# Tzq2doc/distributed_learning_simulator

Hardware: AMD Instinct MI355X
Metric: FL rounds/sec (FedAvg, 100 clients, ResNet-18, CIFAR-10-shaped) (higher is better)
Workload: dtype fp32; 1 GPU; fedavg_resnet18; model=ResNet18, algo=fed_avg, clients=100, local_epochs=5, global_batch=6400, per_client_batch=64, parallelism=client-dp1, backend=hip

## Files before the change

csrc/bindings.cpp:

```cpp
#include <pybind11/pybind11.h>

#include <stdexcept>
#include <string>

#include "dls.h"

namespace py = pybind11;
typedef uintptr_t ptr;

template <typename T>
static T* P(ptr p) {
  return reinterpret_cast<T*>(p);
}
static hipStream_t S(ptr s) { return reinterpret_cast<hipStream_t>(s); }

extern "C" const char* dls_src_hash();

static SgdEpi sgd_arg(const py::object& o) {
  SgdEpi e{};
  if (o.is_none()) return e;
  const py::tuple t = o.cast<py::tuple>();
  if (t.size() != 13) throw std::invalid_argument("sgd epilogue: 13 fields expected");
  e.theta = P<float>(t[0].cast<ptr>());
  e.mom = P<float>(t[1].cast<ptr>());
// ... 7 lines not shown
  e.wd = t[9].cast<float>();
  e.momentum = t[10].cast<float>();
  e.dampening = t[11].cast<float>();
  e.nesterov = t[12].cast<int>();
  return e;
}

PYBIND11_MODULE(_dls_hip, m) {
  m.doc() = "gfx950 kernels for the MI355X-native cohort FL simulator";
  m.def("src_hash", []() { return std::string(dls_src_hash()); });
  m.def("set_native_option", [](const std::string& name, int value) {
    if (!set_native_option(name.c_str(), value)) throw std::invalid_argument("unknown native option " + name);
  });

  m.def("conv_nt", [](ptr x, ptr w, ptr y, ptr bias, long x_cs, long y_cs, long w_cs, long b_cs, int B, int H, int W,
                      int C, int OH, int OW, int KH, int KW, int stride, int pad, int dil, int M, int N, int R, int rep,
                      int relu, int K, int b_kmajor, int variant, ptr acc, ptr gate, int f32, ptr s, int ldx, int ldy,
                      ptr stats, ptr stats_valid, ptr drop_seeds, float drop_p, float out_scale, ptr wsplit,
                      long ws_cs, long ws_plane, long x_lo, ptr yp, long yp_cs, long yp_lo) {
    ConvNTParams p{};
    p.yp = P<bf16_t>(yp);
    p.yp_cs = yp_cs;
    p.yp_lo = yp_lo;
    p.x_lo = x_lo;
    p.wsplit = P<const bf16_t>(wsplit);
    p.ws_cs = ws_cs;
    p.ws_plane = ws_plane;
    p.drop_seeds = P<const uint32_t>(drop_seeds);
    p.drop_p = drop_p;
    p.out_scale = out_scale;
    p.stats = P<float>(stats);
    p.stats_valid = P<const int>(stats_valid);
    p.f32 = f32;
    p.ldx = ldx;
    p.ldy = ldy;
    p.acc = P<const bf16_t>(acc);
    p.gate = P<const bf16_t>(gate);
    p.x = P<const bf16_t>(x);
    p.w = P<const bf16_t>(w);
    p.y = P<bf16_t>(y);
    p.bias = P<const bf16_t>(bias);
    p.x_cs = x_cs; p.y_cs = y_cs; p.w_cs = w_cs; p.b_cs = b_cs;
    p.B = B; p.H = H; p.W = W; p.C = C; p.OH = OH; p.OW = OW; p.KH = KH; p.KW = KW;
    p.stride = stride; p.pad = pad; p.dil = dil; p.M = M; p.N = N; p.R = R; p.rep = rep; p.relu = relu;
    p.b_kmajor = b_kmajor;
    if (stats && stats_valid && native_option(g_opt_halo_skip, "DLS_SKIP_INVALID", 1)) {
      p.skip_valid = P<const int>(stats_valid);
      p.skip_mul = OH * OW;
    }
    conv_nt(p, K, variant, S(s));
  });
  m.def("conv_dgrad", [](ptr dy, ptr w, ptr dx, ptr acc, long w_cs, int K, int rep, int B, int OH, int OW, int Co, int H,
                         int W, int Ci, int KH, int KW, int stride, int pad, int variant, int f32, ptr s, int ld_dy,
                         long dy_cs, ptr wsplit, long ws_cs, long ws_plane, long x_lo, int acc_compact, ptr bnb_part,
                         ptr bnb_x, long bnb_xld, ptr bnb_y, ptr bnb_mask, ptr bnb_mean, ptr bnb_rstd, ptr bnb_valid,
                         ptr wt_buf, ptr acc_mask, int wt_ready) {
    BNBwdPartials bnb{P<float>(bnb_part), P<const float>(bnb_x), bnb_xld, P<const float>(bnb_y),
                      P<const uint8_t>(bnb_mask), P<const float>(bnb_mean), P<const float>(bnb_rstd),
                      P<const int>(bnb_valid)};
    conv_dgrad(P<const bf16_t>(dy), P<const bf16_t>(w), P<bf16_t>(dx), P<const bf16_t>(acc), w_cs, K, rep, B, OH, OW, Co, H, W, Ci, KH, KW,
               stride, pad, variant, f32, S(s), ld_dy, dy_cs, P<const bf16_t>(wsplit), ws_cs, ws_plane, x_lo, acc_compact,
               bnb_part ? &bnb : nullptr, P<bf16_t>(wt_buf), P<const uint8_t>(acc_mask), wt_ready);
  });
  m.def("wt_planes", [](ptr wsplit, long ws_cs, long ws_plane, ptr wt, int Kw, int Co, int Ci, ptr s) {
    wt_planes(P<const bf16_t>(wsplit), ws_cs, ws_plane, P<bf16_t>(wt), Kw, Co, Ci, S(s));
  });
  m.def("conv_gl_wanted", &conv_gl_wanted);
  m.def("conv_gl_fwd", [](ptr x, ptr w, ptr y, ptr bias, long x_cs, long y_cs, long w_cs, long b_cs, int K, int rep,
                          int B, int H, int W, int C, int OH, int OW, int KH, int KW, int stride, int pad, int N,
                          int relu, ptr s) {
    conv_gl_fwd(P<const bf16_t>(x), P<const bf16_t>(w), P<bf16_t>(y), P<const bf16_t>(bias), x_cs, y_cs, w_cs, b_cs,
                K, rep, B, H, W, C, OH, OW, KH, KW, stride, pad, N, relu, S(s));
  });
  m.def("conv_weight_flip_t", [](ptr w, ptr wt, long w_cs, int Kw, int Co, int KH, int KW, int Ci, ptr s) {
    conv_weight_flip_t(P<const bf16_t>(w), P<bf16_t>(wt), w_cs, Kw, Co, KH, KW, Ci, S(s));
  });
  m.def("conv_gl_dgrad", [](ptr dy, ptr wt, ptr dx, ptr acc, int K, int rep, int B, int OH, int OW, int Co, int H, int W,
                            int Ci, int KH, int KW, int stride, int pad, ptr s) {
    conv_gl_dgrad(P<const bf16_t>(dy), P<const bf16_t>(wt), P<bf16_t>(dx), P<const bf16_t>(acc), K, rep, B, OH, OW, Co, H, W, Ci, KH, KW,
                  stride, pad, S(s));
  });
  m.def("conv_nt_num_variants", &conv_nt_num_variants);
  m.def("conv_nt_default_variant", &conv_nt_default_variant);
  m.def("conv_tn", [](ptr dy, ptr x, ptr dw, long dy_cs, long x_cs, long dw_cs, int B, int H, int W, int C, int OH,
                      int OW, int KH, int KW, int stride, int pad, int M, int Co, int R, int K, int variant, int f32,
                      ptr s, int ldy, int ldx, ptr part, long dy_lo, long x_lo, py::object sgd) {
    ConvTNParams p{};
    p.part = P<float>(part);
    p.dy_lo = dy_lo;
    p.x_lo = x_lo;
    p.f32 = f32;
    p.ldy = ldy;
    p.ldx = ldx;
    p.dy = P<const bf16_t>(dy);
    p.x = P<const bf16_t>(x);
    p.dw = P<float>(dw);
    p.dy_cs = dy_cs; p.x_cs = x_cs; p.dw_cs = dw_cs;
    p.B = B; p.H = H; p.W = W; p.C = C; p.OH = OH; p.OW = OW; p.KH = KH; p.KW = KW; p.stride = stride; p.pad = pad;
    p.M = M; p.Co = Co; p.R = R; p.splitk = 1; p.m_per_split = M;
    p.sgd = sgd_arg(sgd);
    conv_tn(p, K, variant, S(s));
  });
  m.def("conv_tn_splitk", &conv_tn_splitk, py::arg("K"), py::arg("Co"), py::arg("R"), py::arg("M"), py::arg("C"),
        py::arg("variant"), py::arg("f32"), py::arg("ldy") = 0, py::arg("ldx") = 0, py::arg("planes") = 0);
  m.def("conv_tn_pl_num_variants", &conv_tn_pl_num_variants);
  m.def("conv_tn_pl_set_variant", &conv_tn_pl_set_variant);
  m.def("conv_tn_pl_variant", &conv_tn_pl_variant);
  m.def("conv_tn_num_variants", &conv_tn_num_variants);
  m.def("conv_nt_f32_num_variants", &conv_nt_f32_num_variants);
  m.def("conv_nt_pl_num_variants", &conv_nt_pl_num_variants);
  m.def("conv_nt_pl_set_variant", &conv_nt_pl_set_variant);
  m.def("conv_halo_set_mode", &conv_halo_set_mode);
  m.def("conv_halo_set_variant", &conv_halo_set_variant);
  m.def("conv_tn_f32_num_variants", &conv_tn_f32_num_variants);

  m.def("bn_workspace_floats", &bn_workspace_floats);
  m.def("bn_fwd", [](ptr x, ptr gamma, ptr beta, ptr res, ptr y, ptr mean, ptr rstd, ptr valid, long g_cs, int K,
                     int R, int C, int relu, float eps, int rep, ptr ws, ptr mask, int f32, ptr s,
                     int ldx, ptr pre_part, int pre_nparts, ptr yp, int y_f32, ptr coef_out, int apply, ptr res_coef) {
    bn_fwd(P<const void>(x), P<const void>(gamma), P<const void>(beta), P<const void>(res), P<void>(y), P<float>(mean),
           P<float>(rstd), P<const int>(valid), g_cs, K, R, C, relu, eps, rep, P<float>(ws), P<uint8_t>(mask),
           f32, S(s), ldx, P<const float>(pre_part), pre_nparts, P<bf16_t>(yp), y_f32,
           P<float>(coef_out), apply, P<const float>(res_coef));
  });
  m.def("conv_halo_bn_supported", &conv_halo_bn_supported);
  m.def("bn_apply_only", [](ptr x, ptr coef, ptr valid, int K, int R, int C, int relu, ptr yp, ptr mask, ptr s, ptr y) {
    bn_apply_only(P<const float>(x), P<const float>(coef), P<const int>(valid), K, R, C, relu, P<bf16_t>(yp),
                  P<uint8_t>(mask), S(s), P<float>(y));
  });
  m.def("conv_halo_bn_fwd", [](ptr x, long x_cs, ptr coef, int relu, ptr valid, ptr wsplit, long ws_cs, long ws_plane,
                               int rep, ptr y, long y_cs, int K, int B, int H, int W, int C, int N, ptr stats,
                               ptr stats_valid, ptr s, ptr yp, ptr mask) {
    return conv_halo_bn_fwd(P<const float>(x), x_cs, P<const float>(coef), relu, P<const int>(valid),
                            P<const bf16_t>(wsplit), ws_cs, ws_plane, rep, P<float>(y), y_cs, K, B, H, W, C, N,
                            P<float>(stats), P<const int>(stats_valid), S(s), P<bf16_t>(yp), P<uint8_t>(mask));
  });
  m.def("bn_coef_sums", [](ptr sums, long sums_cs, int ldp, ptr gamma, ptr beta, ptr valid, long g_cs, int K, int R,
                           int C, float eps, int rep, ptr mean, ptr rstd, ptr coef, ptr s) {
    bn_coef_sums(P<const double>(sums), sums_cs, ldp, P<const float>(gamma), P<const float>(beta), P<const int>(valid),
                 g_cs, K, R, C, eps, rep, P<float>(mean), P<float>(rstd), P<float>(coef), S(s));
  });
  m.def("part_sum_f64", [](ptr part, int K, int nparts, int g, ptr out, long out_cs, int ldo, ptr s) {
    part_sum_f64(P<const float>(part), K, nparts, g, P<double>(out), out_cs, ldo, S(s));
  });
  m.def("chan_sums_f64_ws", &chan_sums_f64_ws);
  m.def("chan_sums_f64", [](ptr x, long x_cs, int ldx, int K, int R, int C, ptr valid, ptr ws, ptr out, long out_cs,
                            int ldo, ptr s) {
    chan_sums_f64(P<const float>(x), x_cs, ldx, K, R, C, P<const int>(valid), P<double>(ws), P<double>(out), out_cs, ldo,
                  S(s));
  });
  m.def("dense_wgrad_supported", &dense_wgrad_supported);
  m.def("dense_wgrad_part_floats", &dense_wgrad_part_floats);
  m.def("dense_wgrad", [](ptr dy, long dy_cs, int ldy, ptr y, long y_cs, ptr dw, long dw_cs, ptr part, int K, int B,
                          int H, int W, int C, int N, ptr s, ptr bn_sc, int ldy_x, ptr valid) {
    return dense_wgrad(P<const float>(dy), dy_cs, ldy, P<const float>(y), y_cs, P<float>(dw), dw_cs, P<float>(part), K, B,
                       H, W, C, N, S(s), P<const float>(bn_sc), ldy_x, P<const int>(valid));
  });
  m.def("dense_dgrad_supported", &dense_dgrad_supported);
  m.def("dense_dgrad_ws_floats", &dense_dgrad_ws_floats);
  m.def("dense_dgrad_bn", [](ptr dy, long dy_cs, int ldy, ptr w, long w_cs, int rep, ptr x, ptr dx, long x_cs, int ldx,
                             ptr mask, ptr y, ptr mean, ptr rstd, ptr valid, ptr gamma, long g_cs, ptr dgamma,
                             ptr dbeta, long dg_cs, ptr ws, int K, int B, int H, int W, int C, int N, ptr s,
                             ptr bn_sc) {
    DenseDgradParams p{};
    p.dy = P<const float>(dy);
    p.dy_cs = dy_cs;
    p.ldy = ldy;
    p.w = P<const float>(w);
    p.w_cs = w_cs;
    p.rep = rep;
    p.x = P<const float>(x);
    p.dx = P<float>(dx);
    p.x_cs = x_cs;
    p.ldx = ldx;
    p.mask = P<const uint8_t>(mask);
    p.y = P<const float>(y);
    p.bn_sc = P<const float>(bn_sc);
    p.mean = P<const float>(mean);
    p.rstd = P<const float>(rstd);
    p.valid_rows = P<const int>(valid);
    p.K = K;
    p.B = B;
    p.H = H;
    p.W = W;
    p.C = C;
    p.N = N;
    return dense_dgrad_bn(p, P<const float>(gamma), g_cs, P<float>(dgamma), P<float>(dbeta), dg_cs, P<float>(ws), S(s));
  });
  m.def("halo_wgrad_supported", &halo_wgrad_supported);
  m.def("halo_wgrad_part_floats", &halo_wgrad_part_floats);
  m.def("halo_wgrad", [](ptr dy, long dy_cs, long dy_lo, int ldy, ptr x, long x_cs, long x_lo, int ldx, ptr coef,
                         int relu, ptr x_valid, ptr dw, long dw_cs, ptr part, int K, int B, int H, int W, int C, int N,
                         int xm, int dm, ptr s, ptr valid_img, py::object sgd, py::object bnb) {
    HaloWgradParams p{};
    p.sgd = sgd_arg(sgd);
    if (!bnb.is_none()) {
      const py::tuple t = bnb.cast<py::tuple>();
      if (t.size() != 5) throw std::invalid_argument("halo_wgrad bnb: 5 fields expected");
      p.bb_x = P<const float>(t[0].cast<ptr>());
      p.bb_mask = P<const uint8_t>(t[1].cast<ptr>());
      p.bb_coef = P<const float>(t[2].cast<ptr>());
      p.bb_valid = P<const int>(t[3].cast<ptr>());
      p.bb_dxp = P<bf16_t>(t[4].cast<ptr>());
    }
    p.valid_img = P<const int>(valid_img);
    p.dy = P<const void>(dy);
    p.dy_cs = dy_cs;
// ... 249 lines not shown
```

csrc/conv_f32.hip:

```cpp
#include "dls.h"
#include "gemm_common.h"
#include "epilogue_f32.h"

#include <numeric>

namespace {

template <int V>
struct FV {
  float v[V];
};

template <int V>
__device__ __forceinline__ void fzero(FV<V>& f) {
#pragma unroll
  for (int i = 0; i < V; ++i) f.v[i] = 0.f;
}

template <int V>
__device__ __forceinline__ void fload(FV<V>& f, const float* p) {
  load_vec<V>(p, f.v);
}

template <int V>
// ... 253 lines not shown
        }
    }
  };

  if constexpr (NBUF == 1) {
    load();
    store(0);
    __syncthreads();
    for (int kt = 0; kt < nk; ++kt) {
      if (kt + 1 < nk) load();
      compute(0);
      if (kt + 1 < nk) {
        __syncthreads();
        store(0);
        __syncthreads();
      }
    }
  } else {
    load();
    store(0);
    __syncthreads();
    int buf = 0;
    for (int kt = 0; kt < nk; ++kt) {
      if (kt + 1 < nk) load();
      compute(buf);
      if (kt + 1 < nk) store(buf ^ 1);
      __syncthreads();
      buf ^= 1;
    }
  }

  nt_f32_epilogue<TM, TN, WM * WN, -1, false>(p, acc, smem, client, m0, n0, wm0, wn0, wid, lane);
}

template <int BM, int BN, int BK, int WM, int WN, int NBUF, int VSET, int MINW = 1>
bool launch_nt_f32_cfg(const ConvNTParams& p, int K, int va, int vb, bool bkm, hipStream_t s) {
  const int grid = K * cdiv(p.M, BM) * cdiv(p.N, BN);
  if (p.wsplit && va == 8 && vb == 8) {
    if (bkm)
      hipLaunchKernelGGL((conv_nt_f32_kernel<BM, BN, BK, WM, WN, 8, 8, true, NBUF, MINW, true>), dim3(grid),
                         dim3(WM * WN * 64), 0, s, p);
    else
      hipLaunchKernelGGL((conv_nt_f32_kernel<BM, BN, BK, WM, WN, 8, 8, false, NBUF, MINW, true>), dim3(grid),
                         dim3(WM * WN * 64), 0, s, p);
    return true;
  }
#define NTF_CASE(A, B)                                                                                       \
  if (va == A && vb == B) {                                                                                  \
    if (bkm)                                                                                                 \
      hipLaunchKernelGGL((conv_nt_f32_kernel<BM, BN, BK, WM, WN, A, B, true, NBUF, MINW>), dim3(grid),             \
                         dim3(WM * WN * 64), 0, s, p);                                                       \
    else                                                                                                     \
      hipLaunchKernelGGL((conv_nt_f32_kernel<BM, BN, BK, WM, WN, A, B, false, NBUF, MINW>), dim3(grid),            \
                         dim3(WM * WN * 64), 0, s, p);                                                       \
    return true;                                                                                             \
  }
  NTF_CASE(8, 8)
  if constexpr (VSET >= 1) { NTF_CASE(4, 4) NTF_CASE(8, 4) NTF_CASE(4, 8) }
  if constexpr (VSET >= 2) { NTF_CASE(8, 1) NTF_CASE(4, 1) NTF_CASE(1, 8) NTF_CASE(1, 4) NTF_CASE(1, 1) }
#undef NTF_CASE
  return false;
}

bool launch_nt_f32_variant(int v, const ConvNTParams& p, int K, int va, int vb, bool bkm, hipStream_t s) {
  switch (v) {
    case 0: return launch_nt_f32_cfg<128, 128, 32, 2, 2, 2, 1>(p, K, va, vb, bkm, s);
    case 1: return launch_nt_f32_cfg<128, 128, 32, 2, 2, 1, 0>(p, K, va, vb, bkm, s);
    case 2: return launch_nt_f32_cfg<256, 128, 32, 4, 2, 1, 0>(p, K, va, vb, bkm, s);
    case 3: return launch_nt_f32_cfg<64, 64, 32, 2, 2, 2, 2>(p, K, va, vb, bkm, s);
    case 4: return launch_nt_f32_cfg<128, 64, 32, 4, 1, 2, 1>(p, K, va, vb, bkm, s);
    case 5: return launch_nt_f32_cfg<128, 128, 64, 2, 2, 1, 0>(p, K, va, vb, bkm, s);
    case 6: return launch_nt_f32_cfg<256, 64, 32, 4, 1, 1, 0>(p, K, va, vb, bkm, s);
    case 7: return launch_nt_f32_cfg<64, 64, 32, 2, 2, 1, 1>(p, K, va, vb, bkm, s);
    case 8: return launch_nt_f32_cfg<128, 128, 32, 2, 2, 1, 0, 3>(p, K, va, vb, bkm, s);
    case 9: return launch_nt_f32_cfg<256, 64, 32, 4, 1, 1, 0, 3>(p, K, va, vb, bkm, s);
    case 10: return launch_nt_f32_cfg<256, 32, 32, 4, 1, 1, 1>(p, K, va, vb, bkm, s);
    default: return false;
  }
}

int vw(int c) { return (c % 8 == 0) ? 8 : (c % 4 == 0) ? 4 : 1; }


template <int BMc, int BNr, int BKT, int WM, int WN, int VA, int VB, int NBUF>
__global__ void __launch_bounds__(WM* WN * 64) conv_tn_f32_kernel(ConvTNParams p) {
  constexpr int T = WM * WN * 64;
  constexpr int TM = BMc / (WM * 32), TN = BNr / (WN * 32);
  constexpr int LDA = BMc + 32;
  constexpr int LDB = BNr + 32;
  constexpr int CCA = BMc / VA, RPA = T / CCA, PA = RPA > BKT ? 1 : BKT / RPA;
  constexpr bool A_PART = RPA > BKT;
  constexpr int CCB = BNr / VB, RPB = T / CCB, PB = BKT / RPB;
  static_assert(PA >= 1 && PB >= 1, "tile too small");
  constexpr int A_PLANE = NBUF * BKT * LDA, B_PLANE = NBUF * BKT * LDB;
  __shared__ __attribute__((aligned(16))) bf16_t smem[2 * (A_PLANE + B_PLANE)];
  bf16_t* const As = smem;
  bf16_t* const Bs = smem + 2 * A_PLANE;

  const int tid = threadIdx.x, lane = tid & 63, wid = tid >> 6;
  const int tilesM = (p.Co + BMc - 1) / BMc, tilesN = (p.R + BNr - 1) / BNr;
  const int per_client = tilesM * tilesN * p.splitk;
  const int bid = xcd_remap(blockIdx.x, gridDim.x);
  const int client = bid / per_client;
  int t = bid % per_client;
  const int split = t % p.splitk;
  t /= p.splitk;
  const int co0 = (t / tilesN) * BMc, r0 = (t % tilesN) * BNr;
  const int mbeg = split * p.m_per_split;
  const int mend = min(p.M, mbeg + p.m_per_split);

  const float* __restrict__ dy = reinterpret_cast<const float*>(p.dy) + (long)client * p.dy_cs;
  const float* __restrict__ x = reinterpret_cast<const float*>(p.x) + (long)client * p.x_cs;

  const int cb = tid % CCB;
  const int rcol = r0 + cb * VB;
  const bool rok = rcol < p.R;
  int kh = 0, kw = 0, c = 0;
  if (rok) {
    kh = rcol / (p.KW * p.C);
    const int rr = rcol - kh * p.KW * p.C;
    kw = rr / p.C;
    c = rr - kw * p.C;
  }
  const int ca = tid % CCA;
  const int cocol = co0 + ca * VA;
  const bool cok = cocol < p.Co;

  FV<VA> ra[PA];
  FV<VB> rb[PB];
  const auto dyr = make_rsrc(dy, (uint32_t)((long)p.M * p.ldy * 4));
  const auto xr = make_rsrc(x, (uint32_t)((long)p.B * p.H * p.W * p.ldx * 4));
  const bool a_live = cok && !(A_PART && tid / CCA >= BKT);
  int k_next = mbeg;
  const int q_b = BKT / (p.OH * p.OW), rem_b = BKT - q_b * p.OH * p.OW;
  const int q_oh = rem_b / p.OW, r_ow = rem_b - q_oh * p.OW;
  const int s_ldx = p.stride * p.ldx, s_row = p.stride * p.W * p.ldx, img = p.H * p.W * p.ldx;
  const int d_iw = r_ow * p.stride, d_off = r_ow * s_ldx + q_oh * s_row + q_b * img;
  const int w_wrap = p.OW * p.stride, off_c1 = s_row - p.OW * s_ldx;
  const int d_ih0 = q_oh * p.stride, d_ih1 = (q_oh + 1) * p.stride;
  const int h_wrap = p.OH * p.stride, off_c2 = img - p.OH * s_row;
  int bx_ow[PB], bx_oh[PB], bx_ih[PB], bx_iw[PB], bx_off[PB];
#pragma unroll
  for (int j = 0; j < PB; ++j) {
    const uint32_t m = mbeg + tid / CCB + j * RPB;
    const uint32_t b = fdiv(m, p.fd_ohw);
    const uint32_t rem = m - b * p.OH * p.OW;
    const uint32_t oh = fdiv(rem, p.fd_ow);
    const uint32_t ow = rem - oh * p.OW;
    bx_ow[j] = ow;
    bx_oh[j] = oh;
    bx_ih[j] = (int)oh * p.stride - p.pad + kh;
    bx_iw[j] = (int)ow * p.stride - p.pad + kw;
    bx_off[j] = (((int)b * p.H + bx_ih[j]) * p.W + bx_iw[j]) * p.ldx + c;
  }
  int a_off = (mbeg + tid / CCA) * p.ldy + cocol;
  const int a_jstep = RPA * p.ldy, a_kstep = BKT * p.ldy;
  auto load = [&]() {
    const int k0 = k_next;
    k_next += BKT;
#pragma unroll
    for (int j = 0; j < PA; ++j) {
      const int m = k0 + tid / CCA + j * RPA;
      buf_load<VA>(ra[j].v, dyr, (a_live && m < mend) ? (uint32_t)(a_off + j * a_jstep) * 4u : OOB_OFF);
    }
    a_off += a_kstep;
#pragma unroll
    for (int j = 0; j < PB; ++j) {
      const int m = k0 + tid / CCB + j * RPB;
      const bool ok = rok && m < mend && (unsigned)bx_ih[j] < (unsigned)p.H && (unsigned)bx_iw[j] < (unsigned)p.W;
      buf_load<VB>(rb[j].v, xr, ok ? (uint32_t)bx_off[j] * 4u : OOB_OFF);
      bx_ow[j] += r_ow;
      bx_iw[j] += d_iw;
      bx_off[j] += d_off;
      const bool c1 = bx_ow[j] >= p.OW;
      bx_ow[j] -= c1 ? p.OW : 0;
      bx_oh[j] += c1 ? q_oh + 1 : q_oh;
      bx_iw[j] -= c1 ? w_wrap : 0;
      bx_ih[j] += c1 ? d_ih1 : d_ih0;
      bx_off[j] += c1 ? off_c1 : 0;
      const bool c2 = bx_oh[j] >= p.OH;
      bx_oh[j] -= c2 ? p.OH : 0;
      bx_ih[j] -= c2 ? h_wrap : 0;
      bx_off[j] += c2 ? off_c2 : 0;
    }
  };
  auto store = [&](int buf) {
#pragma unroll
    for (int j = 0; j < PA; ++j) {
      if (A_PART && tid / CCA >= BKT) continue;
      const int off = (buf * BKT + tid / CCA + j * RPA) * LDA + ca * VA;
      st_split(As + off, As + A_PLANE + off, ra[j]);
    }
#pragma unroll
    for (int j = 0; j < PB; ++j) {
      const int off = (buf * BKT + tid / CCB + j * RPB) * LDB + cb * VB;
      st_split(Bs + off, Bs + B_PLANE + off, rb[j]);
    }
  };

  f32x16 acc[TM][TN];
#pragma unroll
  for (int i = 0; i < TM; ++i)
#pragma unroll
    for (int j = 0; j < TN; ++j) acc[i][j] = f32x16{};

  const int wm0 = (wid / WN) * (TM * 32), wn0 = (wid % WN) * (TN * 32);
  const int g = lane >> 4, q = (lane >> 2) & 3, pp = lane & 3, h = lane >> 5;
  auto compute = [&](int buf) {
#pragma unroll
    for (int ks = 0; ks < BKT / 16; ++ks) {
      bf16x8 ah[TM], al[TM], bh[TN], bl[TN];
      const int krow = buf * BKT + ks * 16 + 8 * h + q;
#pragma unroll
      for (int i = 0; i < TM; ++i) {
        const int o0 = krow * LDA + wm0 + i * 32 + 16 * (g & 1) + 4 * pp, o1 = o0 + 4 * LDA;
        ah[i] = tr_frag(As + o0, As + o1);
        al[i] = tr_frag(As + A_PLANE + o0, As + A_PLANE + o1);
      }
#pragma unroll
      for (int j = 0; j < TN; ++j) {
        const int o0 = krow * LDB + wn0 + j * 32 + 16 * (g & 1) + 4 * pp, o1 = o0 + 4 * LDB;
        bh[j] = tr_frag(Bs + o0, Bs + o1);
        bl[j] = tr_frag(Bs + B_PLANE + o0, Bs + B_PLANE + o1);
      }
#pragma unroll
      for (int i = 0; i < TM; ++i)
#pragma unroll
        for (int j = 0; j < TN; ++j) {
          acc[i][j] = __builtin_amdgcn_mfma_f32_32x32x16_bf16(al[i], bh[j], acc[i][j], 0, 0, 0);
          acc[i][j] = __builtin_amdgcn_mfma_f32_32x32x16_bf16(ah[i], bl[j], acc[i][j], 0, 0, 0);
          acc[i][j] = __builtin_amdgcn_mfma_f32_32x32x16_bf16(ah[i], bh[j], acc[i][j], 0, 0, 0);
        }
    }
  };

  const int nk = (mend - mbeg + BKT - 1) / BKT;
  if (nk <= 0) return;
  if constexpr (NBUF == 1) {
    load();
    store(0);
    __syncthreads();
    for (int kt = 0; kt < nk; ++kt) {
      if (kt + 1 < nk) load();
      compute(0);
      if (kt + 1 < nk) {
        __syncthreads();
        store(0);
        __syncthreads();
      }
    }
  } else {
    load();
    store(0);
    __syncthreads();
    int buf = 0;
    for (int kt = 0; kt < nk; ++kt) {
      if (kt + 1 < nk) load();
      compute(buf);
      if (kt + 1 < nk) store(buf ^ 1);
      __syncthreads();
      buf ^= 1;
    }
  }

  const bool slab = p.splitk > 1 && p.part != nullptr;
  const bool atom = p.splitk > 1 && !slab;
  float* __restrict__ dw = slab ? p.part + ((long)split * (gridDim.x / per_client) + client) * p.Co * p.R
                                : p.dw + (long)client * p.dw_cs;
#pragma unroll
  for (int j = 0; j < TN; ++j) {
    const int r = r0 + wn0 + j * 32 + (lane & 31);
#pragma unroll
    for (int i = 0; i < TM; ++i) {
#pragma unroll
      for (int e = 0; e < 16; ++e) {
        const int co = co0 + wm0 + i * 32 + (e & 3) + 8 * (e >> 2) + 4 * (lane >> 5);
        if (co < p.Co && r < p.R) {
          float* dst = dw + (long)co * p.R + r;
          if (atom)
            atomicAdd(dst, acc[i][j][e]);
          else
            *dst = acc[i][j][e];
        }
      }
    }
  }
}

template <int BMc, int BNr, int BKT, int WM, int WN, int NBUF, bool ALLV>
bool launch_tn_f32_cfg(const ConvTNParams& p, int va, int vb, int grid, hipStream_t s) {
#define TNF_CASE(A, B)                                                                                          \
  if (va == A && vb == B) {                                                                                     \
    hipLaunchKernelGGL((conv_tn_f32_kernel<BMc, BNr, BKT, WM, WN, A, B, NBUF>), dim3(grid), dim3(WM * WN * 64), \
                       0, s, p);                                                                                \
    return true;                                                                                                \
  }
  TNF_CASE(8, 8)
  if constexpr (ALLV) {
    TNF_CASE(4, 4) TNF_CASE(8, 4) TNF_CASE(4, 8) TNF_CASE(1, 1) TNF_CASE(8, 1) TNF_CASE(1, 8) TNF_CASE(4, 1)
    TNF_CASE(1, 4)
  }
#undef TNF_CASE
  return false;
}

struct TnTile {
  int bm, bn;
};
constexpr TnTile kTnF32Tiles[] = {{128, 128}, {64, 128}, {128, 128}, {256, 128}, {128, 256}, {64, 64}, {32, 128},
                                   {64, 256}};
constexpr int kTnF32Variants = sizeof(kTnF32Tiles) / sizeof(kTnF32Tiles[0]);
constexpr int TN_BKT_MAX = 32;

bool launch_tn_f32_variant(int v, const ConvTNParams& p, int va, int vb, int grid, hipStream_t s) {
  switch (v) {
    case 0: return launch_tn_f32_cfg<128, 128, 32, 2, 2, 2, true>(p, va, vb, grid, s);
    case 1: return launch_tn_f32_cfg<64, 128, 32, 2, 2, 2, true>(p, va, vb, grid, s);
    case 2: return launch_tn_f32_cfg<128, 128, 32, 2, 2, 1, false>(p, va, vb, grid, s);
    case 3: return launch_tn_f32_cfg<256, 128, 32, 4, 2, 1, false>(p, va, vb, grid, s);
    case 4: return launch_tn_f32_cfg<128, 256, 32, 2, 4, 1, false>(p, va, vb, grid, s);
    case 5: return launch_tn_f32_cfg<64, 64, 32, 2, 2, 2, true>(p, va, vb, grid, s);
    case 6: return launch_tn_f32_cfg<32, 128, 32, 1, 4, 2, true>(p, va, vb, grid, s);
    case 7: return launch_tn_f32_cfg<64, 256, 32, 2, 2, 1, false>(p, va, vb, grid, s);
    default: return false;
  }
}

int tn_f32_default_variant(int K, int Co, int R) {
  auto tiles = [&](int bm, int bn) { return (long)K * cdiv(Co, bm) * cdiv(R, bn); };
  if (Co <= 32 && R > 64) return 6;
  if (Co <= 32 || R <= 64) return 5;
  (void)tiles;
  if (R <= 256 && Co > 64) return 5;
  if (Co <= 64) return 1;
  if (Co >= 256 && R >= 2048) return 3;
  if (Co >= 1024 && R >= 512) return 3;
  return 0;
}

int resolve_tn_f32_variant(int variant, int K, int Co, int R, int va, int vb) {
  if (variant < 0 || variant >= kTnF32Variants) variant = tn_f32_default_variant(K, Co, R);
  if ((va != 8 || vb != 8) && !(variant == 0 || variant == 1 || variant == 5 || variant == 6))
    variant = Co <= 64 ? 1 : 0;
  return variant;
}

void tn_f32_split(int K, int Co, int R, int M, int variant, int& splitk, int& mps) {
  (void)K;
  const TnTile t = kTnF32Tiles[variant];
  const long tiles = (long)32 * cdiv(Co, t.bm) * cdiv(R, t.bn);
  splitk = 1;
  const int target = 1024;
  if (tiles < target) {
    splitk = (int)((target + tiles - 1) / tiles);
    splitk = min(splitk, max(1, M / (4 * TN_BKT_MAX)));
  }
  mps = cdiv(M, splitk);
  mps = ((mps + TN_BKT_MAX - 1) / TN_BKT_MAX) * TN_BKT_MAX;
  splitk = cdiv(M, mps);
}

}

int conv_nt_f32_num_variants() { return 11; }

void conv_nt_f32(const ConvNTParams& p, int K, int variant, hipStream_t s) {
  if (p.x_lo != 0) {
    if (conv_nt_pl_variant() < 0 && conv_halo(p, K, s)) return;
    if (!conv_nt_pl(p, K, conv_nt_pl_variant(), s)) {
      fprintf(stderr, "conv_nt_f32: pre-split operands in an unsupported shape (C %d, ldx %d, N %d, R %d)\n", p.C,
              p.ldx, p.N, p.R);
      abort();
    }
    return;
  }
  const bool bkm = p.b_kmajor != 0;
  const long xb = (long)p.B * p.H * p.W * p.ldx * 4;
  const long wb = (bkm ? (long)p.C * p.wKH * p.wKW * p.N : (long)p.N * p.R) * 4;
  if (p.dil != 1) {
    fprintf(stderr, "conv_nt_f32: input dilation is not supported\n");
    abort();
  }
  if (xb >= (long)OOB_OFF || wb >= (long)OOB_OFF || (p.wsplit && (p.ws_plane + wb / 4) * 2 >= (long)OOB_OFF)) {
    fprintf(stderr, "conv_nt_f32: per-client operand window over 2 GiB (x %ld B, w %ld B)\n", xb, wb);
    abort();
  }
  const int va = vw(std::gcd(p.C, p.ldx));
  int vb = bkm ? vw(p.N) : vw(p.R);
  if (variant < 0) {
    variant = p.N <= 64 ? 9 : 1;
    if (p.N <= 32) variant = 10;
    if (p.N > 64 && p.KH * p.KW == 1) variant = 8;
  }
  const bool v88 = va == 8 && vb == 8;
  const bool v84 = (va == 8 || va == 4) && (vb == 8 || vb == 4);
  if (!v88) {
    if (!v84 && variant != 3) variant = 3;
    if (v84 && !(variant == 0 || variant == 3 || variant == 4 || variant == 7 || variant == 10))
      variant = p.N <= 64 ? 4 : 0;
  }
  if (!launch_nt_f32_variant(variant, p, K, va, vb, bkm, s)) fprintf(stderr, "conv_nt_f32: bad variant %d\n", variant);
  if (p.yp) {
    if (p.yp_cs != 2 * p.y_cs || p.yp_lo != p.y_cs || p.ldy != p.N || p.out_s != 1) {
      fprintf(stderr, "conv_nt_f32: output planes need contiguous per-client rows\n");
      abort();
    }
    split_rows(reinterpret_cast<const float*>(p.y), p.yp, K, (long)p.M * p.N, p.y_cs, s);
  }
}

int conv_tn_f32_num_variants() { return kTnF32Variants; }

void conv_tn_f32(ConvTNParams p, int K, int variant, hipStream_t s) {
  if (p.sgd.theta && p.dy_lo == 0) {
    fprintf(stderr, "conv_tn_f32: the SGD epilogue needs pre-split operands\n");
    abort();
  }
  if (p.dy_lo != 0) {
    if (!conv_tn_pl(p, K, variant, s)) {
      fprintf(stderr, "conv_tn_f32: pre-split operands in an unsupported shape (C %d, Co %d)\n", p.C, p.Co);
      abort();
    }
    return;
  }
  const long dyb = (long)p.M * (p.ldy ? p.ldy : p.Co) * 4, xb = (long)p.B * p.H * p.W * (p.ldx ? p.ldx : p.C) * 4;
  if (dyb >= (long)OOB_OFF || xb >= (long)OOB_OFF) {
    fprintf(stderr, "conv_tn_f32: per-client operand window over 2 GiB (dy %ld B, x %ld B)\n", dyb, xb);
    abort();
  }
  const int va = vw(std::gcd(p.Co, p.ldy));
  const int vb = vw(std::gcd(p.C, p.ldx));
  variant = resolve_tn_f32_variant(variant, K, p.Co, p.R, va, vb);
  tn_f32_split(K, p.Co, p.R, p.M, variant, p.splitk, p.m_per_split);
  const TnTile t = kTnF32Tiles[variant];
  const long tiles = (long)K * cdiv(p.Co, t.bm) * cdiv(p.R, t.bn);
  const int grid = (int)(tiles * p.splitk);
  if (!launch_tn_f32_variant(variant, p, va, vb, grid, s)) fprintf(stderr, "conv_tn_f32: bad variant %d\n", variant);
  if (p.splitk > 1 && p.part != nullptr) tn_fold(p.part, p.dw, p.dw_cs, K, p.splitk, (long)p.Co * p.R, s);
}

int conv_tn_f32_splitk(int K, int Co, int R, int M, int gco, int gc, int variant) {
  int splitk, mps;
  variant = resolve_tn_f32_variant(variant, K, Co, R, vw(gco), vw(gc));
  tn_f32_split(K, Co, R, M, variant, splitk, mps);
  return splitk;
}
```

csrc/dls.h:

```cpp
#pragma once
#include <hip/hip_runtime.h>
#include <stdint.h>

typedef uint16_t bf16_t;

constexpr int kOptUnset = -1000000;
extern int g_opt_attn_mfma, g_opt_conv_gl, g_opt_pl_min_wg;
extern int g_opt_halo_wgrad_unroll;
extern int g_opt_halo_skip;
extern int g_opt_conv_pix;
int native_option(int& slot, const char* env, int dflt);
bool set_native_option(const char* name, int value);

struct FastDiv {
  uint32_t d, mul, shift;
};

static inline FastDiv make_fastdiv(uint32_t d) {
  FastDiv f;
  f.d = d;
  uint32_t s = 0;
  while ((1u << s) < d) ++s;
  f.shift = s;
  f.mul = (uint32_t)((((uint64_t)1 << 32) * (((uint64_t)1 << s) - d)) / d + 1);
// ... 84 lines not shown
  float* part;
  int K, B, H, W, C, N, nchunks, G;
  const float* bn_sc;
  int ldy_x;
  const int* valid_rows;
};

struct DenseDgradParams {
  const float* dy;
  long dy_cs;
  int ldy;
  const float* w;
  long w_cs;
  int rep;
  const float* x;
  float* dx;
  long x_cs;
  int ldx;
  const uint8_t* mask;
  const float* y;
  const float* bn_sc;
  const float* mean;
  const float* rstd;
  const int* valid_rows;
  const float* coef;
  float* part;
  int K, B, H, W, C, N, G, nchunks;
};

struct SgdEpi {
  float* theta;
  float* mom;
  bf16_t* split;
  long th_cs, sp_cs, sp_lo;
  const float* lr;
  const uint8_t* active;
  const uint8_t* first;
  float wd, momentum, dampening;
  int nesterov;
};

struct HaloWgradParams {
  const void* dy;
  long dy_cs, dy_lo;
  int ldy;
  const void* x;
  long x_cs, x_lo;
  int ldx;
  const float* coef;
  int relu;
  const int* x_valid;
  const int* valid_img;
  const float* bb_x;
  const uint8_t* bb_mask;
  const float* bb_coef;
  const int* bb_valid;
  bf16_t* bb_dxp;
  float* dw;
  long dw_cs;
  float* part;
  int K, B, H, W, C, N;
  int nblk, cblk, G;
  SgdEpi sgd;
};
bool halo_wgrad_supported(int B, int H, int W, int C, int N);
long halo_wgrad_part_floats(int K, int B, int H, int W, int C, int N);
bool halo_wgrad(HaloWgradParams p, int xm, int dm, hipStream_t s);

struct ConvTNParams {
  const bf16_t* dy;
  const bf16_t* x;
  float* dw;
  long dy_cs, x_cs, dw_cs;
  int B, H, W, C, OH, OW, KH, KW, stride, pad;
  int M, Co, R;
  int splitk, m_per_split;
  FastDiv fd_ohw, fd_ow;
  int f32;
  int ldy, ldx;
  float* part;
  long dy_lo, x_lo;
  SgdEpi sgd;
  int pix;
};

struct ConvGLParams {
  const bf16_t* x;
  const bf16_t* w;
  bf16_t* y;
  const bf16_t* bias;
  const bf16_t* acc;
  const bf16_t* zero;
  long x_cs, y_cs, w_cs, b_cs;
  int B, H, W, C;
  int OH, OW;
  int stride, pad_h, pad_w;
  int M, N, ldb, ntaps, cchunks;
  int tap_dh[9], tap_dw[9], tap_boff[9];
  int rep, relu;
  int out_s, out_ph, out_pw, out_H, out_W;
  FastDiv fd_ohw, fd_ow;
};
bool conv_gl_supported(int C, int N, int ntaps);
bool conv_gl_wanted(int K, int M, int N, int C, int ntaps, int mode);
void conv_gl_fwd(const bf16_t* x, const bf16_t* w, bf16_t* y, const bf16_t* bias, long x_cs, long y_cs, long w_cs,
                 long b_cs, int K, int rep, int B, int H, int W, int C, int OH, int OW, int KH, int KW, int stride,
                 int pad, int N, int relu, hipStream_t s);
void conv_weight_flip_t(const bf16_t* w, bf16_t* wt, long w_cs, int Kw, int Co, int KH, int KW, int Ci,
                        hipStream_t s);
void conv_gl_dgrad(const bf16_t* dy, const bf16_t* wt, bf16_t* dx, const bf16_t* acc, int K, int rep, int B, int OH, int OW, int Co,
                   int H, int W, int Ci, int KH, int KW, int stride, int pad, hipStream_t s);

void conv_nt(ConvNTParams p, int K, int variant, hipStream_t s);
int conv_nt_num_variants();
int conv_nt_default_variant(int M, int N, int R, int b_kmajor);
void conv_dgrad(const bf16_t* dy, const bf16_t* w, bf16_t* dx, const bf16_t* acc, long w_cs, int K, int rep, int B, int OH, int OW,
                int Co, int H, int W, int Ci, int KH, int KW, int stride, int pad, int variant, int f32, hipStream_t s,
                int ld_dy = 0, long dy_cs = 0, const bf16_t* wsplit = nullptr, long ws_cs = 0, long ws_plane = 0,
                long x_lo = 0, int acc_compact = 0,
                const BNBwdPartials* bnb = nullptr,
                bf16_t* wt_buf = nullptr,
                const uint8_t* acc_mask = nullptr,
                int wt_ready = 0);
void wt_planes(const bf16_t* wsplit, long ws_cs, long ws_plane, bf16_t* wt, int Kw, int Co, int Ci, hipStream_t s);
void conv_tn(ConvTNParams p, int K, int variant, hipStream_t s);
int conv_tn_num_variants();
int conv_tn_splitk(int K, int Co, int R, int M, int C, int variant, int f32, int ldy = 0, int ldx = 0,
                   int planes = 0);
void conv_nt_f32(const ConvNTParams& p, int K, int variant, hipStream_t s);
int conv_nt_f32_num_variants();
void conv_tn_f32(ConvTNParams p, int K, int variant, hipStream_t s);
bool conv_nt_pl_supported(const ConvNTParams& p);
bool conv_nt_pl(const ConvNTParams& p, int K, int variant, hipStream_t s);
int conv_nt_pl_num_variants();
int conv_nt_pl_variant();
void conv_nt_pl_set_variant(int v);
bool conv_halo(const ConvNTParams& p, int K, hipStream_t s);
bool conv_halo_bn_supported(int B, int H, int W, int C, int N);
void bn_coef_sums(const double* sums, long sums_cs, int ldp, const float* gamma, const float* beta,
                  const int* valid_rows, long g_cs, int K, int R, int C, float eps, int rep, float* mean, float* rstd,
                  float* coef, hipStream_t s);
void part_sum_f64(const float* part, int K, int nparts, int g, double* out, long out_cs, int ldo, hipStream_t s);
long chan_sums_f64_ws(int R, int C);
void chan_sums_f64(const float* x, long x_cs, int ldx, int K, int R, int C, const int* valid, double* ws, double* out,
                   long out_cs, int ldo, hipStream_t s);
void bn_apply_only(const float* x, const float* coef, const int* valid_rows, int K, int R, int C, int relu,
                   bf16_t* yp, uint8_t* rmask, hipStream_t s, float* y = nullptr);
bool conv_halo_bn_fwd(const float* x, long x_cs, const float* coef, int relu, const int* valid_rows,
                      const bf16_t* wsplit, long ws_cs, long ws_plane, int rep, float* y, long y_cs, int K, int B,
                      int H, int W, int C, int N, float* stats, const int* stats_valid, hipStream_t s,
                      bf16_t* yp = nullptr, uint8_t* mask = nullptr);
bool conv_halo_bn_dense_supported(int B, int H, int W, int C, int N);
bool conv_halo_bn_dense_fwd(const float* x, long x_cs, int ldx, int creal, const float* coef, int relu,
                            const int* valid_rows, const bf16_t* wsplit, long ws_cs, long ws_plane, int rep, float* y,
                            long y_cs, int ldy, int K, int B, int H, int W, int C, int N, float* stats,
                            const int* stats_valid, float* ny, long ny_cs, int ldny, uint8_t* mask, hipStream_t s);
bool dense_dgrad_supported(int B, int H, int W, int C, int N);
long dense_dgrad_ws_floats(int K, int B, int H, int C);
bool dense_dgrad_bn(DenseDgradParams p, const float* gamma, long g_cs, float* dgamma, float* dbeta, long dg_cs,
                    float* ws, hipStream_t s);
void bn_bwd_coef_parts(const float* part, int nparts, const float* gamma, long g_cs, const int* valid_rows,
                       const float* mean, const float* rstd, int K, int R, int C, float* coef, float* dgamma,
                       float* dbeta, long dg_cs, hipStream_t s);
bool dense_wgrad_supported(int B, int H, int W, int C, int N);
long dense_wgrad_part_floats(int K, int B, int H, int W, int C);
bool dense_wgrad(const float* dy, long dy_cs, int ldy, const float* y, long y_cs, float* dw, long dw_cs, float* part,
                 int K, int B, int H, int W, int C, int N, hipStream_t s, const float* bn_sc = nullptr,
                 int ldy_x = 0, const int* valid_rows = nullptr);
void conv_halo_set_mode(int m);
void conv_halo_set_variant(int v);
bool conv_tn_pl_supported(const ConvTNParams& p);
bool conv_tn_pl(ConvTNParams p, int K, int variant, hipStream_t s);
int conv_tn_pl_num_variants();
int conv_tn_pl_variant();
void conv_tn_pl_set_variant(int v);
int conv_tn_pl_splitk(int K, int Co, int R, int M, int variant);
void tn_fold(const float* part, float* dw, long dw_cs, int K, int splitk, long CoR, hipStream_t s,
             const SgdEpi* sgd = nullptr);
int conv_tn_f32_num_variants();
int conv_tn_f32_splitk(int K, int Co, int R, int M, int gco, int gc, int variant);

long bn_workspace_floats(int K, long R, int C);
void bn_fwd(const void* x, const void* gamma, const void* beta, const void* res, void* y, float* mean, float* rstd,
            const int* valid_rows, long g_cs, int K, int R, int C, int relu, float eps, int rep, float* ws,
            uint8_t* relu_mask, int f32, hipStream_t s,
            int ldx = 0, const float* pre_part = nullptr,
            int pre_nparts = 0, bf16_t* yp = nullptr,
            int y_f32 = 1, float* coef_out = nullptr, int apply = 1,
            const float* res_coef = nullptr);
void bn_bwd(const void* dy, const void* x, const void* y, const float* mean, const float* rstd, const void* gamma,
            const int* valid_rows, long g_cs, int K, int R, int C, int relu, void* dx, void* dpre, float* dgamma,
            float* dbeta, long dg_cs, float* ws, const uint8_t* relu_mask, int f32,
            hipStream_t s, int ldx = 0,
            int acc_dx = 0, bf16_t* dxp = nullptr,
            int dx_f32 = 1,
            const float* pre_part = nullptr,
            int pre_nparts = 0,
            float* coef_ext = nullptr,
            int stage = 0);
void ln_fwd(const void* x, const void* gamma, const void* beta, void* y, float* mean, float* rstd, long g_cs, int K,
            long rows_per_client, int C, float eps, int rep, int f32, hipStream_t s,
            bf16_t* yp = nullptr);
void ln_bwd(const void* dy, const void* x, const float* mean, const float* rstd, const void* gamma, long g_cs, int K,
            long rows_per_client, int C, void* dx, float* dgamma, float* dbeta, long dg_cs, float* ws, int f32,
            hipStream_t s);
long col_sum_workspace_floats(int K, long rows, int C);
long ln_workspace_floats(int K, long rows_per_client, int C);
void col_sum(const void* x, float* out, long out_cs, int K, long rows, int C, int f32, hipStream_t s,
             float* ws = nullptr);

void pool_fwd(const void* x, void* y, int* idx, int K, int B, int H, int W, int C, int OH, int OW, int k, int stride,
              int pad, int mode, int f32, hipStream_t s);
void pool_bwd(const void* dy, const int* idx, void* dx, int K, int B, int H, int W, int C, int OH, int OW, int k,
              int stride, int pad, int mode, int f32, hipStream_t s);
void gap_fwd(const void* x, void* y, int KB, int HW, int C, int f32, hipStream_t s);
void gap_bwd(const void* dy, void* dx, int KB, int HW, int C, int f32, hipStream_t s);
void ce_fwd_bwd(const void* logits, const int* labels, const int* valid, float* loss, float* correct, void* dlogits,
                int K, int B, int NC, int f32, hipStream_t s, float* rowbuf = nullptr);
void relu_bwd(const void* dy, const void* y, void* dx, long n, int f32, hipStream_t s);

void quant_pack(const float* x, long ld, const int* seg, const int64_t* seg_off, const int64_t* seg_numel,
                const uint8_t* bits, const float* lo, const float* scale, const int64_t* seg_byte_off,
                const int64_t* row_off, int K, int nseg, long P, int stochastic, const uint32_t* seeds, uint8_t* out,
                hipStream_t s);
void quant_unpack(const uint8_t* codes, const int* seg, const int64_t* seg_off, const int64_t* seg_numel,
                  const uint8_t* bits, const float* lo, const float* scale, const int64_t* seg_byte_off,
                  const int64_t* row_off, int K, int nseg, long P, float* out, long ld, hipStream_t s);
void quant_unpack_acc(const uint8_t* codes, const int* seg, const int64_t* seg_off, const int64_t* seg_numel,
                      const uint8_t* bits, const float* lo, const float* scale, const int64_t* seg_byte_off,
                      const int64_t* row_off, int K, int nseg, long P, const double* w, double* acc, hipStream_t s);

#define TOPK_CHUNK 4096
void topk_pack(const float* delta, long ld_d, float* u, long ld_u, int ef, const uint32_t* vbits, uint32_t* hist,
               uint32_t* state, uint32_t* cnt, uint32_t* excl, int* idx, float* val, int K, long P, int k,
               hipStream_t s);
void topk_decode(const int* idx, const float* val, float* out, long ld, int K, long P, int k, hipStream_t s);
void topk_accumulate(const int* idx, const float* val, const double* w, double* acc, int K, long P, int k,
                     hipStream_t s);

#define TRIM_MAX_ROWS 512
void trimmed_sum(const float* x, long ld, int n, int b, long P, double* out, hipStream_t s);

#define PAIR_SPAN 4096
#define PAIR_GROUP 8
int pairwise_spans_per_wg(int n, long P);
long pairwise_ws_doubles(int n, long P, int spw);
void pairwise_sq_dists(const float* x, long ld, int n, long P, double* ws, int spw, double* out, hipStream_t s);

void dropout_apply(const void* x, void* out, int K, long rows, int N, long ld, const uint32_t* seeds, float p,
                   float scale, int f32, hipStream_t s);
long dropout_planes_ws_floats(int K, long rows, int N);
void dropout_planes(const float* x, float* out, bf16_t* yp, int K, long rows, int N, const uint32_t* seeds, float p,
                    float scale, hipStream_t s, float* colsum = nullptr, long colsum_cs = 0, float* ws = nullptr);
void fold_col_partials(const float* part, int nparts, int C, float* out, long out_cs, int K, hipStream_t s);

void synth_images(const int64_t* idx, long n, long npix, int C, int Cout, const int* source, const float* proto,
                  unsigned long long salt, float sqrt6, float noise, float* out, hipStream_t s);

void neighbor_sample(const int* rowptr, const int* col, const int* owner, const uint8_t* is_val, const int64_t* nodes,
                     const int64_t* clients, int n, int fanout, unsigned long long seed_h, int* out_nbr, int* out_cnt,
                     hipStream_t s);

void sgd_step(float* theta, const float* grad, float* mom, bf16_t* shadow, bf16_t* split, const float* lr,
              const uint8_t* active,
              const uint8_t* first, int K, long P, long ld, float wd, float momentum, float dampening, int nesterov,
              hipStream_t s);
void sgd_step_seg(float* theta, const float* grad, float* mom, bf16_t* split, const float* lr, const uint8_t* active,
                  const uint8_t* first, int K, long ld, float wd, float momentum, float dampening, int nesterov,
                  const long2* seg, int nblocks, hipStream_t s);
void adam_step(float* theta, const float* grad, float* m, float* v, bf16_t* shadow, const float* lr,
               const uint8_t* active, const float* step, int K, long P, long ld, float b1, float b2, float eps,
               float wd, hipStream_t s);
// ... 50 lines not shown
```

csrc/norm.hip:

```cpp
#include "common.h"
#include <algorithm>
#include <numeric>

#include "dls.h"

namespace {

constexpr int ROWS_PER_BLOCK = 512;

static int rows_per_block(long R, int K) {
  const long want = std::min<long>(64, (2048 + K - 1) / K);
  const long bpc = std::max(1L, std::min(want, std::max(1L, R / 64)));
  return (int)std::min<long>(ROWS_PER_BLOCK, (R + bpc - 1) / bpc);
}

struct BNCoefArgs {
  const void* gamma;
  const void* beta;
  const float* mean_in;
  const float* rstd_in;
  float* mean_out;
  float* rstd_out;
  float* coef;
  float* dgamma;
// ... 244 lines not shown
  if (c < C) {
    const int lp = ldp ? ldp : C;
    const PT* part = ws + (long)k * (pcs ? pcs : (long)nparts * 2 * lp);
    for (int b = grp; b < nparts; b += G) {
      d0 += part[(long)b * 2 * lp + c];
      d1 += part[(long)b * 2 * lp + lp + c];
    }
  }
  red[0][grp][cl] = d0;
  red[1][grp][cl] = d1;
  __syncthreads();
  if (grp != 0 || c >= C) return;
#pragma unroll
  for (int g2 = 1; g2 < G; ++g2) {
    d0 += red[0][g2][cl];
    d1 += red[1][g2][cl];
  }
  const float s0 = (float)d0, s1 = (float)d1;
  const long i = (long)k * C + c;
  const int nvalid = valid_rows ? min(valid_rows[k], R) : R;
  const float n = (float)max(nvalid, 1);
  const float g = ldf(gamma + (long)(k / rep) * g_cs + c);
  if (!bwd) {
    const double mud = d0 / n;
    const float mu = (float)mud;
    const float var = (float)fmax(d1 / n - mud * mud, 0.0);
    const float rs = rsqrtf(var + eps);
    const float sc = g * rs;
    mean_out[i] = mu;
    rstd_out[i] = rs;
    coef[2 * i] = sc;
    coef[2 * i + 1] = ldf(beta + (long)(k / rep) * g_cs + c) - mu * sc;
  } else {
    const float mu = mean_in[i], rs = rstd_in[i];
    const float a = g * rs;
    const float e = -a * rs * s1 / n;
    const float d = -a * s0 / n - e * mu;
    coef[3 * i] = a;
    coef[3 * i + 1] = d;
    coef[3 * i + 2] = e;
    if (dgamma) {
      dbeta[(long)k * dg_cs + c] = s0;
      dgamma[(long)k * dg_cs + c] = s1;
    }
  }
}

template <typename TT, typename PT, typename... A>
void launch_coef(dim3 grid, hipStream_t s, A... args) {
  hipLaunchKernelGGL((bn_coef_kernel<TT, PT, 8>), grid, dim3(32 * 8), 0, s, args...);
}

template <int V>
__device__ __forceinline__ void store_planes(bf16_t* hi, bf16_t* lo, const float* f) {
  if constexpr (V % 2 == 0) {
    uint32_t h[V / 2], l[V / 2];
#pragma unroll
    for (int i = 0; i < V / 2; ++i) split_pair(f[2 * i], f[2 * i + 1], h[i], l[i]);
    if constexpr (V == 8) {
      *reinterpret_cast<uint4*>(hi) = make_uint4(h[0], h[1], h[2], h[3]);
      *reinterpret_cast<uint4*>(lo) = make_uint4(l[0], l[1], l[2], l[3]);
    } else if constexpr (V == 4) {
      *reinterpret_cast<uint2*>(hi) = make_uint2(h[0], h[1]);
      *reinterpret_cast<uint2*>(lo) = make_uint2(l[0], l[1]);
    } else {
#pragma unroll
      for (int i = 0; i < V / 2; ++i) {
        reinterpret_cast<uint32_t*>(hi)[i] = h[i];
        reinterpret_cast<uint32_t*>(lo)[i] = l[i];
      }
    }
  } else {
#pragma unroll
    for (int i = 0; i < V; ++i) split2(f[i], hi[i], lo[i]);
  }
}

template <typename T, int V>
__global__ void __launch_bounds__(256) bn_apply_kernel(const T* __restrict__ x, const T* __restrict__ res,
                                                       T* __restrict__ y, const int* __restrict__ valid_rows,
                                                       const float* __restrict__ coef, int R, int C, int relu,
                                                       int rpb, uint8_t* __restrict__ rmask, int ldx,
                                                       bf16_t* __restrict__ yp, int y_f32,
                                                       const float* __restrict__ res_coef) {
  const int k = blockIdx.y;
  const int CT = C / V;
  const int nvalid = valid_rows ? min(valid_rows[k], R) : R;
  const int r0 = blockIdx.x * rpb, r1 = min(R, r0 + rpb);
  const long base = (long)k * R * C, base_x = (long)k * R * ldx;
  for (int cg = 0; cg < CT; cg += 256) {
    const int ctn = min(256, CT - cg);
    const int RT = 256 / ctn;
    const int cc = threadIdx.x % ctn, rl = threadIdx.x / ctn;
    if (rl >= RT) continue;
    const int c0 = (cg + cc) * V;
    float sc[V], sh[V], rsc[V], rsh[V];
#pragma unroll
    for (int j = 0; j < V; ++j) {
      sc[j] = coef[2 * ((long)k * C + c0 + j)];
      sh[j] = coef[2 * ((long)k * C + c0 + j) + 1];
      rsc[j] = res_coef ? res_coef[2 * ((long)k * C + c0 + j)] : 0.f;
      rsh[j] = res_coef ? res_coef[2 * ((long)k * C + c0 + j) + 1] : 0.f;
    }
    for (int r = r0 + rl; r < r1; r += RT) {
      const long off = base + (long)r * C + c0;
      float out[V];
      if (r < nvalid) {
        float v[V];
        const long offx = base_x + (long)r * ldx + c0;
        load_vec<V>(x + offx, v);
#pragma unroll
        for (int j = 0; j < V; ++j) out[j] = fmaf(v[j], sc[j], sh[j]);
        if (res) {
          float rv[V];
          load_vec<V>(res + offx, rv);
          if (res_coef) {
#pragma unroll
            for (int j = 0; j < V; ++j) out[j] += fmaf(rv[j], rsc[j], rsh[j]);
          } else {
#pragma unroll
            for (int j = 0; j < V; ++j) out[j] += rv[j];
          }
        }
        if (relu) {
#pragma unroll
          for (int j = 0; j < V; ++j) out[j] = fmaxf(out[j], 0.f);
        }
      } else {
#pragma unroll
        for (int j = 0; j < V; ++j) out[j] = 0.f;
      }
      if (rmask) {
        uint32_t m = 0;
#pragma unroll
        for (int j = 0; j < V; ++j) m |= (rt<T>(out[j]) > 0.f ? 1u : 0u) << j;
        rmask[((long)k * R + r) * (C / 8) + c0 / 8] = (uint8_t)m;
      }
      if (y_f32) store_vec<V>(y + off, out);
      if (yp) {
        bf16_t* hp = yp + (long)k * R * C + off;
        store_planes<V>(hp, hp + (long)R * C, out);
      }
    }
  }
}

template <typename T, int V>
__global__ void __launch_bounds__(256) bn_bwd_apply_kernel(const T* __restrict__ dy, const T* __restrict__ x,
                                                           const T* __restrict__ y,
                                                           const int* __restrict__ valid_rows,
                                                           const float* __restrict__ coef, int R, int C, int relu,
                                                           T* __restrict__ dx, T* __restrict__ dpre,
                                                           int rpb, const uint8_t* __restrict__ rmask, int ldx,
                                                           int acc_dx, bf16_t* __restrict__ dxp, int dx_f32) {
  const int k = blockIdx.y;
  const int CT = C / V;
  const int nvalid = valid_rows ? min(valid_rows[k], R) : R;
  const int r0 = blockIdx.x * rpb, r1 = min(R, r0 + rpb);
  const long base = (long)k * R * C, base_x = (long)k * R * ldx;
  for (int cg = 0; cg < CT; cg += 256) {
    const int ctn = min(256, CT - cg);
    const int RT = 256 / ctn;
    const int cc = threadIdx.x % ctn, rl = threadIdx.x / ctn;
    if (rl >= RT) continue;
    const int c0 = (cg + cc) * V;
    float ca[V], cd[V], ce[V];
#pragma unroll
    for (int j = 0; j < V; ++j) {
      const long q = 3 * ((long)k * C + c0 + j);
      ca[j] = coef[q];
      cd[j] = coef[q + 1];
      ce[j] = coef[q + 2];
    }
    for (int r = r0 + rl; r < r1; r += RT) {
      const long off = base + (long)r * C + c0;
      const long offx = base_x + (long)r * ldx + c0;
      float o[V], gp[V];
      if (r < nvalid) {
        float vdy[V], vx[V];
        load_vec<V>(dy + off, vdy);
        load_vec<V>(x + offx, vx);
        if (rmask) {
          const uint32_t mbits = rmask[((long)k * R + r) * (C / 8) + c0 / 8];
#pragma unroll
          for (int j = 0; j < V; ++j) vdy[j] = ((mbits >> j) & 1u) ? vdy[j] : 0.f;
        } else if (relu) {
          float vy[V];
          load_vec<V>(y + off, vy);
#pragma unroll
          for (int j = 0; j < V; ++j) vdy[j] = vy[j] > 0.f ? vdy[j] : 0.f;
        }
#pragma unroll
        for (int j = 0; j < V; ++j) {
          gp[j] = vdy[j];
          o[j] = fmaf(ca[j], vdy[j], fmaf(ce[j], vx[j], cd[j]));
        }
      } else {
#pragma unroll
        for (int j = 0; j < V; ++j) o[j] = gp[j] = 0.f;
// ... 157 lines not shown
    b = wave_sum(b) / C;
#pragma unroll
    for (int i = 0; i < NC; ++i) {
      const int c = lane + 64 * i;
      if (c < C) stf(dx + row * C + c, crs * (cy[i] * gv[i] - a - xh[i] * b));
    }
#pragma unroll
    for (int i = 0; i < NC; ++i) {
      cy[i] = ny[i];
      cx[i] = nx[i];
    }
    cmu = nmu;
    crs = nrs;
  }
  if (rend > rbeg || part) {
#pragma unroll
    for (int i = 0; i < NC; ++i) {
      const int c = lane + 64 * i;
      if (c < C) {
        if (part) {
          float* pw = part + ((long)k * gridDim.x * 4 + wave) * 2 * C;
          pw[c] = dg[i];
          pw[C + c] = db[i];
        } else {
          atomicAdd(&dgamma[(long)k * dg_cs + c], dg[i]);
          atomicAdd(&dbeta[(long)k * dg_cs + c], db[i]);
        }
      }
    }
  }
}

__global__ void __launch_bounds__(256) part_sum_kernel(const float* __restrict__ part, int nparts, int W, int C,
                                                       float* __restrict__ out0, float* __restrict__ out1, long out_cs) {
  const int k = blockIdx.y, c = blockIdx.x * 256 + threadIdx.x;
  if (c >= C) return;
  const float* p = part + (long)k * nparts * W;
  float a = 0.f, b = 0.f;
  for (int i = 0; i < nparts; ++i) {
    a += p[(long)i * W + c];
    if (out1) b += p[(long)i * W + C + c];
  }
  out0[(long)k * out_cs + c] = a;
  if (out1) out1[(long)k * out_cs + c] = b;
}

}

#define DISPATCH_V(V, ...)          \
  if (V == 8) {                     \
    constexpr int VV = 8;           \
    __VA_ARGS__;                    \
  } else if (V == 4) {              \
    constexpr int VV = 4;           \
    __VA_ARGS__;                    \
  } else {                          \
    constexpr int VV = 1;           \
    __VA_ARGS__;                    \
  }
#define DISPATCH_T(F32, ...)        \
  if (F32) {                        \
    typedef float TT;               \
    __VA_ARGS__;                    \
  } else {                          \
    typedef bf16_t TT;              \
    __VA_ARGS__;                    \
  }
#define CP(p) static_cast<const TT*>(p)
#define MP(p) static_cast<TT*>(p)

static long bn_fold_offset(int K, long R, int C) {
  const long parts = (R + rows_per_block(R, K) - 1) / rows_per_block(R, K);
  return ((long)K * 3 * C + (long)K * parts * 2 * C + 1) & ~1L;
}

long bn_workspace_floats(int K, long R, int C) {
  const long nfold = cdiv((int)cdiv((int)R, 32), FOLD);
  return bn_fold_offset(K, R, C) + (long)K * nfold * 2 * C * 2;
}

void bn_fwd(const void* x, const void* gamma, const void* beta, const void* res, void* y, float* mean, float* rstd,
            const int* valid_rows, long g_cs, int K, int R, int C, int relu, float eps, int rep, float* ws,
            uint8_t* rmask, int f32, hipStream_t s, int ldx, const float* pre_part,
            int pre_nparts, bf16_t* yp, int y_f32, float* coef_out, int apply, const float* res_coef) {
  if (ldx == 0) ldx = C;
  float* coef = coef_out ? coef_out : ws;
  const float* part = pre_part ? pre_part : ws + (long)3 * C * K;
  const int rpb = rows_per_block(R, K);
  dim3 grid(cdiv(R, rpb), K);
  const int nparts = pre_part ? pre_nparts : (int)grid.x;
  const int V = vw(std::gcd(C, ldx));
  BNCoefArgs ca{gamma, beta, nullptr, nullptr, mean, rstd, coef, nullptr, nullptr, 0L, g_cs, eps, rep, 0};
  if (V != 8) rmask = nullptr;
  DISPATCH_T(f32, {
    if (!pre_part) {
      DISPATCH_V(V, hipLaunchKernelGGL((chan_reduce_kernel<TT, VV, 0>), grid, dim3(256), 0, s, CP(x), nullptr, nullptr,
                                       nullptr, nullptr, valid_rows, R, C, 0, ws + (long)3 * C * K, (long)2 * C, rpb,
                                       nullptr, ca, ldx, ldx));
    }
    if (pre_part && nparts > FOLD && nparts <= cdiv(R, 32)) {
      const int nfold = cdiv(nparts, FOLD);
      double* folds = reinterpret_cast<double*>(ws + bn_fold_offset(K, R, C));
      hipLaunchKernelGGL(part_fold_kernel, dim3(nfold, K), dim3(256), 0, s, pre_part, nparts, 2 * C, folds, nfold);
      launch_coef<TT, double>(dim3(cdiv(C, 32), K), s, (const double*)folds, nfold, CP(gamma), CP(beta), valid_rows,
                              (const float*)nullptr, (const float*)nullptr, mean, rstd, coef, (float*)nullptr,
                              (float*)nullptr, 0L, g_cs, K, R, C, eps, rep, 0, 0, 0L);
    } else {
      launch_coef<TT, float>(dim3(cdiv(C, 32), K), s, part, nparts, CP(gamma), CP(beta), valid_rows,
                             (const float*)nullptr, (const float*)nullptr, mean, rstd, coef, (float*)nullptr,
                             (float*)nullptr, 0L, g_cs, K, R, C, eps, rep, 0, 0, 0L);
    }
    if (apply) {
      DISPATCH_V(V, hipLaunchKernelGGL((bn_apply_kernel<TT, VV>), grid, dim3(256), 0, s, CP(x), CP(res), MP(y),
                                       valid_rows, coef, R, C, relu, rpb, rmask, ldx, f32 ? yp : nullptr,
                                       f32 ? y_f32 : 1, res_coef));
    }
  });
}

void bn_apply_only(const float* x, const float* coef, const int* valid_rows, int K, int R, int C, int relu,
                   bf16_t* yp, uint8_t* rmask, hipStream_t s, float* y) {
  const int rpb = rows_per_block(R, K);
  dim3 grid(cdiv(R, rpb), K);
  if (C % 8 == 0) {
    hipLaunchKernelGGL((bn_apply_kernel<float, 8>), grid, dim3(256), 0, s, x, (const float*)nullptr, y,
                       valid_rows, coef, R, C, relu, rpb, rmask, C, yp, y ? 1 : 0, (const float*)nullptr);
  } else {
    hipLaunchKernelGGL((bn_apply_kernel<float, 1>), grid, dim3(256), 0, s, x, (const float*)nullptr, y,
                       valid_rows, coef, R, C, relu, rpb, (uint8_t*)nullptr, C, yp, y ? 1 : 0, (const float*)nullptr);
  }
}

void bn_bwd(const void* dy, const void* x, const void* y, const float* mean, const float* rstd, const void* gamma,
            const int* valid_rows, long g_cs, int K, int R, int C, int relu, void* dx, void* dpre, float* dgamma,
            float* dbeta, long dg_cs, float* ws, const uint8_t* rmask, int f32, hipStream_t s,
            int ldx, int acc_dx, bf16_t* dxp, int dx_f32, const float* pre_part, int pre_nparts, float* coef_ext,
            int stage) {
  if (!f32 || acc_dx || (ldx != 0 && ldx != C)) {
    dxp = nullptr;
    dx_f32 = 1;
  }
  if (ldx == 0) ldx = C;
  float* coef = coef_ext ? coef_ext : ws;
  float* part = ws + (long)3 * C * K;
  const int rpb = rows_per_block(R, K);
  dim3 grid(cdiv(R, rpb), K);
  const int V = vw(std::gcd(C, ldx));
  if (V != 8) rmask = nullptr;
  BNCoefArgs ca{gamma, nullptr, mean, rstd, nullptr, nullptr, coef, dgamma, dbeta, dg_cs, g_cs, 0.f, 1, 1};
  DISPATCH_T(f32, {
    if (stage == 2) {
    } else if (pre_part) {
      if (pre_nparts > FOLD && pre_nparts <= cdiv(R, 32)) {
        const int nfold = cdiv(pre_nparts, FOLD);
        double* folds = reinterpret_cast<double*>(ws + bn_fold_offset(K, R, C));
        hipLaunchKernelGGL(part_fold_kernel, dim3(nfold, K), dim3(256), 0, s, pre_part, pre_nparts, 2 * C, folds,
                           nfold);
        launch_coef<TT, double>(dim3(cdiv(C, 32), K), s, (const double*)folds, nfold, CP(gamma), (const TT*)nullptr,
                                valid_rows, mean, rstd, (float*)nullptr, (float*)nullptr, coef, dgamma, dbeta, dg_cs,
                                g_cs, K, R, C, 0.f, 1, 1, 0, 0L);
      } else {
        launch_coef<TT, float>(dim3(cdiv(C, 32), K), s, pre_part, pre_nparts, CP(gamma), (const TT*)nullptr,
                               valid_rows, mean, rstd, (float*)nullptr, (float*)nullptr, coef, dgamma, dbeta, dg_cs,
                               g_cs, K, R, C, 0.f, 1, 1, 0, 0L);
      }
    } else {
      DISPATCH_V(V, hipLaunchKernelGGL((chan_reduce_kernel<TT, VV, 1>), grid, dim3(256), 0, s, CP(dy), CP(x), CP(y),
                                       mean, rstd, valid_rows, R, C, relu, part, (long)2 * C, rpb, rmask, ca, C, ldx));
    }
    if (!pre_part && stage != 2)
      launch_coef<TT, float>(dim3(cdiv(C, 32), K), s, (const float*)part, (int)grid.x, CP(gamma), (const TT*)nullptr,
                             valid_rows, mean, rstd, (float*)nullptr, (float*)nullptr, coef, dgamma, dbeta, dg_cs, g_cs, K,
                             R, C, 0.f, 1, 1, 0, 0L);
    if (stage != 1)
      DISPATCH_V(V, hipLaunchKernelGGL((bn_bwd_apply_kernel<TT, VV>), grid, dim3(256), 0, s, CP(dy), CP(x), CP(y),
                                       valid_rows, coef, R, C, relu, MP(dx), MP(dpre), rpb, rmask, ldx, acc_dx, dxp,
                                       dx_f32));
  });
}

void fold_col_partials(const float* part, int nparts, int C, float* out, long out_cs, int K, hipStream_t s) {
  hipLaunchKernelGGL(part_sum_kernel, dim3(cdiv(C, 256), K), dim3(256), 0, s, part, nparts, C, C, out, (float*)nullptr,
                     out_cs);
}

void bn_bwd_coef_parts(const float* part, int nparts, const float* gamma, long g_cs, const int* valid_rows,
                       const float* mean, const float* rstd, int K, int R, int C, float* coef, float* dgamma,
                       float* dbeta, long dg_cs, hipStream_t s) {
  launch_coef<float, float>(dim3(cdiv(C, 32), K), s, part, nparts, gamma, (const float*)nullptr, valid_rows, mean, rstd,
                            (float*)nullptr, (float*)nullptr, coef, dgamma, dbeta, dg_cs, g_cs, K, R, C, 0.f, 1, 1, 0,
                            0L);
}

void part_sum_f64(const float* part, int K, int nparts, int g, double* out, long out_cs, int ldo, hipStream_t s) {
  if (K == 0) return;
  hipLaunchKernelGGL(part_sum_f64_kernel<float>, dim3(K), dim3(1024), 0, s, part, nparts, g, out, out_cs, ldo);
}

long chan_sums_f64_ws(int R, int C) { return (long)cdiv(R, 256) * 2 * C; }

void chan_sums_f64(const float* x, long x_cs, int ldx, int K, int R, int C, const int* valid, double* ws, double* out,
                   long out_cs, int ldo, hipStream_t s) {
  if (K == 0 || R == 0) return;
  const int rb = 256, nch = cdiv(R, rb);
  hipLaunchKernelGGL(chan_sums_f64_kernel, dim3(nch, K), dim3(256), 0, s, x, x_cs, ldx, R, C, valid, rb, ws, nch);
  hipLaunchKernelGGL(part_sum_f64_kernel<double>, dim3(K), dim3(1024), 0, s, (const double*)ws, nch, C, out, out_cs,
                     ldo);
}

void bn_coef_sums(const double* sums, long sums_cs, int ldp, const float* gamma, const float* beta,
                  const int* valid_rows, long g_cs, int K, int R, int C, float eps, int rep, float* mean, float* rstd,
                  float* coef, hipStream_t s) {
// ... 74 lines not shown
```

distributed_learning_simulator_amd/models/zoo.py:

```python

from __future__ import annotations

import math

import torch

from ..engine.params import ParamLayout
from ..ops import functional as Fn
from .layers import (AvgPool, BatchNorm, Conv2d, Embedding, conv_bn, Flatten, LayerNorm, Linear,
                     MaxPool, Module, ReLU, RunCtx, Seq)


class CohortModel:

    def __init__(self, root: Module, name: str, input_kind: str, num_classes: int):
        self.root = root
        self.name = name
        self.input_kind = input_kind
        self.num_classes = num_classes
        root.assign_names("")
        self.layout = ParamLayout()
        root.register(self.layout)

    def forward(self, x, ctx: RunCtx):
# ... 55 lines not shown
        return Fn.ResidualLink()
    return None


def _down(seq: Seq, x, ctx, donor=None):
    conv, bn = seq.children
    return conv_bn(conv, bn, x, ctx, conv_donor=donor, planes=4)


class BasicBlock(Module):
    kind = "BasicBlock"
    expansion = 1

    def __init__(self, cin, cout, stride):
        super().__init__()
        self.child("conv1", Conv2d(cin, cout, 3, stride, 1))
        self.child("bn1", BatchNorm(cout, relu=True))
        self.child("conv2", Conv2d(cout, cout, 3, 1, 1))
        self.child("bn2", BatchNorm(cout))
        self.down = None
        if stride != 1 or cin != cout:
            self.down = self.child("downsample", Seq(Conv2d(cin, cout, 1, stride, 0), BatchNorm(cout)))

    def forward(self, x, ctx, out_planes: int = 1):
        link = _residual_link(self, x, ctx)
        out = conv_bn(self.conv1, self.bn1, x, ctx, conv_link=link, planes=3)
        sc = x if self.down is None else _down(self.down, x, ctx, donor=link)
        return conv_bn(self.conv2, self.bn2, out, ctx, residual=sc, relu=True,
                       link=link if self.down is None else None, planes=out_planes)


class Bottleneck(Module):
    kind = "Bottleneck"
    expansion = 4

    def __init__(self, cin, width, stride):
        super().__init__()
        cout = width * 4
        self.child("conv1", Conv2d(cin, width, 1, 1, 0))
        self.child("bn1", BatchNorm(width, relu=True))
        self.child("conv2", Conv2d(width, width, 3, stride, 1))
        self.child("bn2", BatchNorm(width, relu=True))
        self.child("conv3", Conv2d(width, cout, 1, 1, 0))
        self.child("bn3", BatchNorm(cout))
        self.down = None
        if stride != 1 or cin != cout:
            self.down = self.child("downsample", Seq(Conv2d(cin, cout, 1, stride, 0), BatchNorm(cout)))

    def forward(self, x, ctx, out_planes: int = 1):
        link = _residual_link(self, x, ctx)
        out = conv_bn(self.conv1, self.bn1, x, ctx, conv_link=link, planes=2)
        out = conv_bn(self.conv2, self.bn2, out, ctx, planes=2)
        sc = x if self.down is None else _down(self.down, x, ctx, donor=link)
        return conv_bn(self.conv3, self.bn3, out, ctx, residual=sc, relu=True,
                       link=link if self.down is None else None, planes=out_planes)


class ResNetNet(Module):
    kind = "ResNet"

    def __init__(self, block, layers, classes=10, cin=3, cifar_stem=True):
        super().__init__()
        self.cifar_stem = cifar_stem
        if cifar_stem:
            self.child("conv1", Conv2d(cin, 64, 3, 1, 1))
        else:
            self.child("conv1", Conv2d(cin, 64, 7, 2, 3))
        self.child("bn1", BatchNorm(64, relu=True))
        if not cifar_stem:
            self.child("maxpool", MaxPool(3, 2, 1))
        c = 64
        self.stages = []
        for i, (n, w) in enumerate(zip(layers, (64, 128, 256, 512))):
            blocks = []
            for j in range(n):
                stride = 2 if (j == 0 and i > 0) else 1
                b = block(c, w, stride)
                blocks.append(b)
                c = w * block.expansion
            self.stages.append(self.child(f"layer{i + 1}", Seq(*blocks)))
        self.child("fc", Linear(c, classes))

    def forward(self, x, ctx):
        x = conv_bn(self.conv1, self.bn1, x, ctx, planes=0 if not self.cifar_stem else 1)
        if not self.cifar_stem:
            x = self.maxpool.forward(x, ctx)
        blocks = [b for s in self.stages for b in s.children]
        for i, b in enumerate(blocks):
            nxt = blocks[i + 1] if i + 1 < len(blocks) else None
            op = 0 if nxt is None else 2 if nxt.down is not None else 1
            x = b.forward(x, ctx, out_planes=op)
        x = Fn.global_avg_pool(x)
        return self.fc.forward(x, ctx)


class DenseLayer(Module):

    kind = "DenseLayer"

    def __init__(self, cin, growth):
        super().__init__()
        self.child("norm", BatchNorm(cin, relu=True))
        self.child("relu", ReLU())
        self.child("conv", Conv2d(cin, growth, 3, 1, 1))

    def forward(self, x, ctx):
        y = self.conv.forward(self.norm.forward(x, ctx), ctx)
        return torch.cat([x, y], dim=-1)


class Transition(Module):
    kind = "Transition"

    def __init__(self, cin, cout):
        super().__init__()
        self.child("norm", BatchNorm(cin, relu=True))
        self.child("relu", ReLU())
        self.child("conv", Conv2d(cin, cout, 1, 1, 0))
        self.child("pool", AvgPool(2))

    def forward(self, x, ctx):
        return self.pool.forward(self.conv.forward(self.norm.forward(x, ctx), ctx), ctx)


class DenseBlock(Seq):

    kind = "Sequential"

    def __init__(self, layers, growth):
        super().__init__(*layers)
        self.growth = growth

    def forward(self, x, ctx):
        P = ctx.P
        lps = [Fn.DenseLayerParams(P.w(l.norm.gamma), P.w(l.norm.beta), P.g(l.norm.gamma), P.g(l.norm.beta),
                                   P.w(l.conv.w), P.g(l.conv.w)) for l in self.children]
        rps = x.shape[2] * x.shape[3]
        return Fn.dense_block(x, ctx.token, lps, self.growth, ctx.valid_rows(rps), training=ctx.training)


class DenseNetNet(Module):
    kind = "DenseNet"

    def __init__(self, depth=40, growth=12, classes=10, cin=3):
        super().__init__()
        n = (depth - 4) // 3
        c = 2 * growth
        self.child("conv1", Conv2d(cin, c, 3, 1, 1))
        self.blocks = []
        for b in range(3):
            layers = []
            for _ in range(n):
                layers.append(DenseLayer(c, growth))
                c += growth
            self.blocks.append(self.child(f"dense{b + 1}", DenseBlock(layers, growth)))
            if b < 2:
                self.blocks.append(self.child(f"trans{b + 1}", Transition(c, c)))
        self.child("norm", BatchNorm(c, relu=True))
        self.child("relu", ReLU())
        self.child("fc", Linear(c, classes))

    def forward(self, x, ctx):
        x = self.conv1.forward(x, ctx)
        for b in self.blocks:
            x = b.forward(x, ctx)
        x = self.norm.forward(x, ctx)
        x = Fn.global_avg_pool(x)
        return self.fc.forward(x, ctx)


# ... 220 lines not shown
```

distributed_learning_simulator_amd/ops/functional.py:

```python

from __future__ import annotations

import collections

import torch

from ..options import OPTIONS
from . import backend, ref


def _be(t):
    return backend.get(t)


class ResidualLink:

    __slots__ = ("grad", "receiver_done", "compact", "receiver_stride")

    def __init__(self):
        self.grad = None
        self.receiver_done = False
        self.compact = 0
        self.receiver_stride = 1


class MaskedGrad:

    __slots__ = ("dy", "mask")

    def __init__(self, dy, mask):
        self.dy, self.mask = dy, mask

    def dense(self):
        K, C = self.dy.shape[0], self.dy.shape[-1]
        bits = torch.arange(8, device=self.mask.device, dtype=torch.uint8)
        keep = ((self.mask.view(K, -1, C // 8, 1) >> bits) & 1).reshape(K, -1, C).bool()
        return torch.where(keep, self.dy.reshape(K, -1, C), torch.zeros((), dtype=self.dy.dtype,
                                                                          device=self.dy.device)).view(self.dy.shape)




class BNStats:

    __slots__ = ("valid", "part", "dy_planes_ok")

    def __init__(self, valid=None):
        self.valid = valid
        self.part = None
        self.dy_planes_ok = False


bn_bwd_parts_count = {"used": 0, "none": 0, "fallback": 0}


class BNBwdLink:

    __slots__ = ("x", "mask", "mean", "rstd", "valid", "part", "key")

    def __init__(self, x, mask, mean, rstd, valid):
        self.x, self.mask, self.mean, self.rstd, self.valid = x, mask, mean, rstd, valid
        self.part = None
        self.key = None

    def args(self, part):
        return (part, self.x, self.mask, self.mean, self.rstd, self.valid, None)




def _planes_of(t):
    return getattr(t, "_dls_planes", None)


def _tag_planes(t, planes, only: bool):
    t._dls_planes = planes
    t._dls_planes_only = only
    return t


def _require_fp32(t, who: str):
    if getattr(t, "_dls_planes_only", False):
        raise RuntimeError(f"{who}: a planes-only activation reached an op that reads fp32 values")


class DeferredBN:

    __slots__ = ("x", "coef", "relu", "valid_rows", "yp", "mask", "write_out", "pending")

    def __init__(self, x, coef, relu, valid_rows, yp, mask, write_out):
        self.x, self.coef, self.relu, self.valid_rows = x, coef, relu, valid_rows
        self.yp, self.mask, self.write_out = yp, mask, write_out
        self.pending = True

    def materialize(self):
        if self.pending:
            from . import hip

            hip.bn_apply_only(self.x, self.coef, self.valid_rows, self.relu, self.yp, self.mask)
            self.pending = False


res_fold_count = {"folded": 0, "materialized": 0}


class DeferredRes:

    __slots__ = ("x", "coef", "valid_rows", "y", "pending")

    def __init__(self, x, coef, valid_rows, y):
        self.x, self.coef, self.valid_rows, self.y = x, coef, valid_rows, y
        self.pending = True

    def materialize(self):
        if self.pending:
            from . import hip

            hip.bn_apply_only(self.x, self.coef, self.valid_rows, False, None, y=self.y)
            self.pending = False
            res_fold_count["materialized"] += 1


bn_bwd_defer_count = {"wgrad": 0, "materialized": 0}


class DeferredBNBwd:

    __slots__ = ("dy", "x", "mask", "coef", "valid_rows", "dxp", "pending")

    def __init__(self, dy, x, mask, coef, valid_rows, dxp):
        self.dy, self.x, self.mask, self.coef, self.valid_rows, self.dxp = dy, x, mask, coef, valid_rows, dxp
        self.pending = True

    def materialize(self):
        if self.pending:
            from . import hip

            hip.bn_bwd_apply_planes(self.dy, self.x, self.mask, self.coef, self.valid_rows, self.dxp)
            self.pending = False
            bn_bwd_defer_count["materialized"] += 1

    def wgrad_args(self):
        return (self.dy, self.x, self.mask, self.coef, self.valid_rows, self.dxp)


class _Conv(torch.autograd.Function):

    @staticmethod
    def forward(ctx, x, token, w, gw, stride, pad, b, gb, link=None, stats=None, w_split=None, donor=None,
                sgd=None):
        be = _be(x)
        ci = w.shape[-1]
        ctx.sgd = sgd if (sgd is not None and be is not ref and x.dtype == torch.float32 and gw is not None
                          and b is None and x.shape[-1] == ci and w_split is not None) else None
        if x.shape[-1] > ci:
            w = torch.nn.functional.pad(w, (0, x.shape[-1] - ci))
            w_split = None
        if be is ref or x.dtype != torch.float32:
            w_split = None
        xp = _planes_of(x)
        use_pl = (xp is not None and w_split is not None and x.is_contiguous()
                  and be.conv_planes_ok(x.shape[-1], w.shape[1]) and be.planes_fit(x[0].numel()))
        if getattr(x, "_dls_planes_only", False) and not use_pl:
            raise RuntimeError("conv2d: planes-only input but the split-plane GEMM cannot run here")
        pl = {"x_planes": xp} if use_pl else {}
        ctx.xp = xp if use_pl else None
        if stats is not None:
            stats.dy_planes_ok = use_pl and b is None
        K, B, H, W = x.shape[:4]
        KH = w.shape[2]
        OH, OW = (H + 2 * pad - KH) // stride + 1, (W + 2 * pad - w.shape[3]) // stride + 1
        y_numel = B * OH * OW * w.shape[1]
        big = be is not ref and max(x[0].numel(), y_numel) * x.element_size() >= (1 << 31)
        if stats is not None:
            stats.dy_planes_ok = stats.dy_planes_ok and be.planes_fit(y_numel)
        want_stats = stats is not None and be is not ref and x.dtype == torch.float32 and not big
        y = None
        ctx.bn_src = None
        defer = getattr(x, "_dls_bn_defer", None)
        if defer is not None and defer.pending:
            if (use_pl and stride == 1 and pad == 1 and KH == 3 and w.shape[3] == 3 and b is None
                    and be.halo_bn_ok(x.shape, w)):
                part = (torch.empty((K, be.conv_stats_parts(B * OH * OW), 2, w.shape[1]), dtype=torch.float32,
                                    device=x.device) if want_stats else None)
                bn_wgrad = (defer.write_out and gw is not None and OPTIONS.halo_wgrad
                            and x.shape[-1] == ci and be.halo_wgrad_ok(x.shape, w.shape[1]))
                y = be.conv_halo_bn_fwd(defer.x.view(x.shape), defer.coef, defer.relu, defer.valid_rows, w, w_split,
                                        stats=part, stats_valid=stats.valid if want_stats else None,
                                        yp=defer.yp if defer.write_out and not bn_wgrad else None,
                                        mask=defer.mask if defer.write_out else None)
                if y is not None:
                    defer.pending = False
                    if want_stats:
                        stats.part = part
                    if bn_wgrad:
                        ctx.bn_src = (defer.x.view(x.shape), defer.coef, defer.relu, defer.valid_rows)
            defer.materialize()
        if y is not None:
            pass
        elif want_stats:
            stats.part = torch.empty((K, be.conv_stats_parts(B * OH * OW), 2, w.shape[1]), dtype=torch.float32,
                                     device=x.device)
            y = be.conv_fwd(x, w, stride, pad, bias=b, stats=stats.part, stats_valid=stats.valid,
                            **({"w_split": w_split} if w_split is not None else {}), **pl)
        elif w_split is not None:
            y = be.conv_fwd(x, w, stride, pad, bias=b, w_split=w_split, **pl)
        else:
            y = be.conv_fwd(x, w, stride, pad, bias=b)
        ctx.w_split = w_split
        ctx.expect_dy_planes = stats is not None and stats.dy_planes_ok
        ctx.x_planes_only = bool(getattr(x, "_dls_planes_only", False))
        bnb = getattr(x, "_dls_bnb", None) if OPTIONS.bn_bwd_parts else None
        if bnb is not None and not (be is not ref and donor is None and x.shape[-1] == ci and not big
                                    and be.bn_bwd_parts_ok(x.shape, stride, x.dtype)):
            bnb = None
        ctx.bnb = bnb
        ctx.halo_wgrad = OPTIONS.halo_wgrad
        ctx.valid = stats.valid if (stats is not None and OPTIONS.skip_invalid) else None
        ctx.dgrad_wt = be is not ref
        ctx.save_for_backward(x, w)
        ctx.gw, ctx.gb, ctx.stride, ctx.pad, ctx.ci = gw, gb, stride, pad, ci
        ctx.link = link
        ctx.donor = donor
        if link is not None:
            link.receiver_stride = stride
        return y

    @staticmethod
    def _wgrad(ctx, dy, x, w, dyp, be, bbd=None, sgd_ok=True) -> bool:
        if bbd is not None:
            if not (ctx.stride == 1 and ctx.pad == 1 and w.shape[2] == 3 and w.shape[3] == 3):
                return False
            sgd = ctx.sgd if sgd_ok else None
            if ctx.bn_src is not None:
                xr, coef, relu, vrows = ctx.bn_src
                ok = be.halo_wgrad(dy, xr, ctx.gw, bn=(coef, relu, vrows), valid=ctx.valid, sgd=sgd,
                                   bn_bwd=bbd.wgrad_args())
            else:
                ok = be.halo_wgrad(dy, x, ctx.gw, x_planes=ctx.xp, valid=ctx.valid, sgd=sgd, bn_bwd=bbd.wgrad_args())
            if ok and sgd is not None:
                sgd[0].done.add(sgd[1])
            return bool(ok)
        padded = w.shape[-1] > ctx.ci
        K = x.shape[0]
        sgd = ctx.sgd if not padded else None
        stepped = False
        gw = torch.empty((K,) + tuple(w.shape[1:]), dtype=torch.float32, device=dy.device) if padded else ctx.gw
        if be is ref:
            gw.copy_(ref.conv_wgrad(dy.float(), x.float(), (K,) + tuple(w.shape[1:]), ctx.stride, ctx.pad))
            if ctx.gb is not None:
                ctx.gb.copy_(dy.float().sum(dim=(1, 2, 3)))
        elif ctx.bn_src is not None:
            xr, coef, relu, vrows = ctx.bn_src
            if not be.halo_wgrad(dy, xr, gw, dy_planes=dyp, bn=(coef, relu, vrows), valid=ctx.valid,
                                 sgd=sgd):
                raise RuntimeError("conv2d backward: the halo wgrad refused a shape its forward accepted")
            stepped = sgd is not None
        elif (ctx.halo_wgrad and ctx.stride == 1 and ctx.pad == 1 and w.shape[2] == 3 and w.shape[3] == 3
              and not padded and be.halo_wgrad(dy, x, gw, dy_planes=dyp, x_planes=ctx.xp, valid=ctx.valid,
                                               sgd=sgd)):
            stepped = sgd is not None
        elif dyp is not None:
            stepped = be.conv_wgrad(dy, x, gw, ctx.stride, ctx.pad, dy_planes=dyp, x_planes=ctx.xp, sgd=sgd)
        else:
            if ctx.x_planes_only:
                raise RuntimeError("conv2d backward: fp32 dY with a planes-only input")
            be.conv_wgrad(dy, x, gw, ctx.stride, ctx.pad)
            if ctx.gb is not None:
                be.bias_grad(dy, ctx.gb)
        if padded:
            ctx.gw.copy_(gw[..., : ctx.ci])
        if stepped:
            sgd[0].done.add(sgd[1])
        return True

    @staticmethod
    def backward(ctx, dy):
        x, w = ctx.saved_tensors
        be = _be(dy)
        dy = dy.contiguous()
        dx = None
        link = ctx.link
        acc = link.grad if link is not None else None
        acc_mask = None
        if isinstance(acc, MaskedGrad):
            if be is not ref and dy.dtype == torch.float32 and ctx.needs_input_grad[0] and not link.compact:
                acc, acc_mask = acc.dy.contiguous(), acc.mask
            else:
                acc = acc.dense()
        acc_compact = False
        if link is not None:
            if acc is not None and link.compact:
                if link.compact == ctx.stride and ctx.stride > 1 and be is not ref and ctx.needs_input_grad[0]:
                    acc_compact = True
                else:
                    full = torch.zeros(x.shape, dtype=acc.dtype, device=acc.device)
                    full[:, :, :: link.compact, :: link.compact] = acc
                    acc = full
            link.grad = None
            link.compact = 0
            if acc is None:
                link.receiver_done = True
        dyp = _planes_of(dy)
        wgrad_done = False
        wt_pre = None
        bbd = getattr(dy, "_dls_bnbwd", None)
        if bbd is not None and bbd.pending:
            if ctx.gw is not None and be is not ref and ctx.halo_wgrad and w.shape[-1] == ctx.ci:
                sgd_ok = True
                if ctx.sgd is not None and ctx.needs_input_grad[0]:
                    wt_pre = (be.dgrad_wt_prebuild(dy.shape, w, ctx.w_split, x.shape[2:4], ctx.stride, ctx.pad)
                              if ctx.dgrad_wt and ctx.w_split is not None and not acc_compact and ctx.donor is None
                              else None)
                    sgd_ok = wt_pre is not None
                wgrad_done = _Conv._wgrad(ctx, dy, x, w, dyp, be, bbd, sgd_ok=sgd_ok)
            if wgrad_done:
                bbd.pending = False
                bn_bwd_defer_count["wgrad"] += 1
            else:
                bbd.materialize()
        if dyp is not None and ctx.xp is None:
            raise RuntimeError("conv2d backward: dY planes without the input's planes")
        if dyp is None:
            if ctx.expect_dy_planes:
                raise RuntimeError("conv2d backward: the BN wrote dY as planes only, but they did not arrive")
            _require_fp32(dy, "conv2d backward")
        donor = ctx.donor
        compact = (donor is not None and not donor.receiver_done and be is not ref and dy.dtype == torch.float32
                   and ctx.stride > 1 and ctx.pad == 0 and w.shape[2] == 1 and w.shape[3] == 1 and acc is None
                   and w.shape[-1] == ctx.ci and donor.receiver_stride == ctx.stride)
        if ctx.needs_input_grad[0] and compact:
            dx = be.conv_dgrad(dy, w, dy.shape[2:4], 1, 0, w_split=ctx.w_split,
                               **({"dy_planes": dyp} if dyp is not None else {}))
        elif ctx.needs_input_grad[0]:
            if acc_compact:
                dx = be.conv_dgrad(dy, w, x.shape[2:4], ctx.stride, ctx.pad, acc=acc, w_split=ctx.w_split,
                                   acc_compact=True, **({"dy_planes": dyp} if dyp is not None else {}))
            else:
                kw = {}
                bnb = ctx.bnb
                if bnb is not None:
                    K, B, H, W, Ci = x.shape
                    part = torch.empty((K, be.conv_stats_parts(B * H * W), 2, Ci), dtype=torch.float32,
                                       device=dy.device)
                    kw["bnb"] = bnb.args(part)
                if dyp is not None:
                    kw["dy_planes"] = dyp
                if ctx.w_split is not None:
                    kw["w_split"] = ctx.w_split
                if acc_mask is not None:
                    kw["acc_mask"] = acc_mask
                if ctx.dgrad_wt:
                    kw["wt"] = True
                if wt_pre is not None:
                    kw["wt_buf"] = wt_pre
                dx = be.conv_dgrad(dy, w, x.shape[2:4], ctx.stride, ctx.pad, acc=acc, **kw)
                if bnb is not None:
                    bnb.part, bnb.key = part, (dx.data_ptr(), dx._version)
            if dx.shape[-1] > ctx.ci:
                dx = dx[..., : ctx.ci]
        elif acc is not None:
            dx = acc if acc_mask is None else MaskedGrad(acc, acc_mask).dense()
        if ctx.gw is not None and not wgrad_done:
            _Conv._wgrad(ctx, dy, x, w, dyp, be)
        if donor is not None and dx is not None and not donor.receiver_done:
            donor.grad = dx
            donor.compact = ctx.stride if compact else 0
            dx = None
        return dx, None, None, None, None, None, None, None, None, None, None, None, None


def conv2d(x, token, w, gw, stride=1, pad=0, b=None, gb=None, link: ResidualLink | None = None,
           stats: BNStats | None = None, w_split: torch.Tensor | None = None, donor: ResidualLink | None = None,
           sgd=None):
    if link is not None:
        assert w.shape[-1] == x.shape[-1], "a residual link needs an unpadded conv"
    return _Conv.apply(x, token, w, gw, stride, pad, b, gb, link, stats, w_split, donor, sgd)


class _Linear(torch.autograd.Function):

    @staticmethod
    def forward(ctx, x, token, w, b, gw, gb, residual=None, relu=False, premasked=False, gate_input=False,
                drop_p=0.0, drop_seeds=None, gate_scale=1.0, w_split=None, x_planes=None, out_planes=False,
                dx_planes=False, res_link=None, acc_link=None, sgd=None):
        be = _be(x)
        ctx.res_link, ctx.acc_link = res_link, acc_link
        shp = x.shape
        x = x.reshape(shp[0], -1, shp[-1])
        ctx.res_shape = residual.shape if residual is not None else None
        if residual is not None:
            residual = residual.reshape(shp[0], x.shape[1], -1).contiguous()
        native = be is not ref and x.dtype == torch.float32 and w_split is not None and OPTIONS.planes
        if not native:
            w_split = x_planes = None
            out_planes = dx_planes = False
        if not OPTIONS.tfm_planes:
            out_planes = dx_planes = False
        ws = {"w_split": w_split} if w_split is not None else {}
        xp = {"x_planes": x_planes} if x_planes is not None else {}
        y = be.linear_fwd(x, w, b, relu=relu, acc=residual, drop_p=drop_p, drop_seeds=drop_seeds, **ws, **xp,
                          **({"out_planes": True} if out_planes else {}))
        yp = None
        if out_planes:
            y, yp = y
        ctx.ws = ws
        mask_dy = relu and not premasked
        ctx.save_for_backward(x, w, y if mask_dy else None, drop_seeds if drop_p else None)
        ctx.x_planes = x_planes
# ... 54 lines not shown
            if dyp is not None:
                kw["dy_planes"] = dyp
            if ctx.dx_planes:
                kw["out_planes"] = True
            if acc is not None and be is not ref:
                kw["acc"] = acc.reshape(K, N, Fi)
            dx = be.linear_dgrad(dy, w, gate=gate, gate_scale=ctx.gate_scale, **kw)
            dxp = None
            if ctx.dx_planes:
                dx, dxp = dx
            if acc is not None and be is ref:
                dx = dx + acc.reshape(dx.shape)
            dx = dx.view(ctx.shape)
            if dxp is not None:
                _tag_planes(dx, dxp.view((K, 2) + tuple(ctx.shape[1:])), False)
        if ctx.gw is not None:
            if be is ref:
                dw, db = ref.linear_wgrad(dy.float(), x.float(), ctx.gb is not None)
                ctx.gw.copy_(dw)
                if ctx.gb is not None:
                    ctx.gb.copy_(db)
            else:
                pl = {"dy_planes": dyp, "x_planes": ctx.x_planes} if (dyp is not None and ctx.x_planes is not None) else {}
                if pl and ctx.sgd is not None:
                    pl["sgd"] = ctx.sgd
                if be.linear_wgrad(dy, x, ctx.gw, None if bias_done else ctx.gb, **pl):
                    ctx.sgd[0].done.add(ctx.sgd[1])
        if dx is None and acc is not None:
            dx = acc.reshape(ctx.shape)
        return (dx, None, None, None, None, None, dres, None, None, None, None, None, None, None, None, None, None, None,
                None, None)


def linear(x, token, w, b, gw, gb, residual=None, relu=False, premasked=False, gate_input=False,
           drop_p: float = 0.0, drop_seeds=None, gate_scale: float = 1.0, w_split=None, out_planes: bool = False,
           dx_planes: bool = False, res_link: ResidualLink | None = None, acc_link: ResidualLink | None = None,
           sgd=None):
    assert not (relu and residual is not None), "ReLU and residual epilogues are not combined"
    return _Linear.apply(x, token, w, b, gw, gb, residual, relu, premasked, gate_input, drop_p, drop_seeds,
                         gate_scale, w_split, _planes_of(x), out_planes, dx_planes, res_link, acc_link, sgd)


class _LinearSharedInput(torch.autograd.Function):

    @staticmethod
    def forward(ctx, x, token, w, gw):
        be = _be(x)
        K, Fo, Fi = w.shape
        wcat = w.reshape(1, K * Fo, Fi).contiguous()
        y = be.linear_fwd(x.unsqueeze(0).contiguous(), wcat, None)
        ctx.save_for_backward(x)
        ctx.gw, ctx.K, ctx.Fo = gw, K, Fo
        return y[0].view(-1, K, Fo).permute(1, 0, 2).contiguous()

    @staticmethod
    def backward(ctx, dy):
        (x,) = ctx.saved_tensors
        if ctx.gw is not None:
            be = _be(dy)
            K, Fo = ctx.K, ctx.Fo
            dyc = dy.permute(1, 0, 2).reshape(1, -1, K * Fo).contiguous()
            Fi = x.shape[-1]
            if be is ref:
                dw, _ = ref.linear_wgrad(dyc.float(), x.unsqueeze(0).float(), False)
            else:
                dw = torch.empty((1, K * Fo, Fi), dtype=torch.float32, device=dy.device)
                be.linear_wgrad(dyc, x.unsqueeze(0).contiguous(), dw, None)
            ctx.gw.copy_(dw.view(K, Fo, Fi))
        return None, None, None, None


def linear_shared_input(x, token, w, gw):
    return _LinearSharedInput.apply(x, token, w, gw)


class _BN(torch.autograd.Function):
    @staticmethod
    def forward(ctx, x, token, gamma, beta, ggamma, gbeta, valid_rows, relu, residual, link=None, stats=None,
                planes=0):
        be = _be(x)
        K = x.shape[0]
        C = x.shape[-1]
        _require_fp32(x, "batch_norm")
        if residual is not None:
            _require_fp32(residual, "batch_norm residual")
        x3 = x.reshape(K, -1, C)
        r3 = residual.reshape(K, -1, C) if residual is not None else None
        mask = None
        yp = None
        bnb = None
        res_coef = None
        fold = getattr(residual, "_dls_res_fold", None) if residual is not None else None
        if fold is not None and fold.pending:
            if (be is not ref and x.dtype == torch.float32 and fold.valid_rows is valid_rows
                    and fold.x.shape == x3.shape and x3.is_contiguous()):
                r3, res_coef = fold.x, fold.coef
                fold.pending = False
                res_fold_count["folded"] += 1
            else:
                fold.materialize()
        fold_out = None
        if be is ref:
            y, mean, rstd = be.bn_fwd(x3, gamma, beta, valid_rows, relu, r3)
        else:
            pre = stats.part if stats is not None else None
            planes = planes if (OPTIONS.planes and x.dtype == torch.float32 and x.is_contiguous()
                                and be.planes_fit(x[0].numel())) else 0
            wm = any(ctx.needs_input_grad)
            C8 = C % 8 == 0
            if planes == 3 and not (OPTIONS.bn_fused_halo and residual is None and C8 and x3.is_contiguous()):
                planes = 2
            if planes == 4 and not (OPTIONS.bn_res_fold and residual is None and not relu and x3.is_contiguous()):
                planes = 0
            if planes == 4:
                coef, mean, rstd = be.bn_coef(x3, gamma, beta, valid_rows, pre_stats=pre)
                y = torch.empty((K, x3.shape[1], C), dtype=x.dtype, device=x.device)
                fold_out = DeferredRes(x3, coef, valid_rows, y)
                defer = None
                planes = 0
            elif planes == 3:
                coef, mean, rstd = be.bn_coef(x3, gamma, beta, valid_rows, pre_stats=pre)
                y, yp = be.planes_buffer((K, x3.shape[1], C), x.device)
                mask = torch.empty((K, x3.shape[1], C // 8), dtype=torch.uint8, device=x.device) if (wm and relu) else None
                defer = DeferredBN(x3, coef, relu, valid_rows, yp, mask, write_out=wm)
            else:
                defer = None
                out = be.bn_fwd(x3, gamma, beta, valid_rows, relu, r3, with_mask=wm, pre_stats=pre, planes=planes,
                                res_coef=res_coef)
                y, mean, rstd = out[:3]
                mask = out[3] if wm else None
                if planes:
                    yp = out[-1]
            if stats is not None:
                stats.part = None
            if (wm and OPTIONS.bn_bwd_parts and x.dtype == torch.float32 and x3.is_contiguous()
                    and (mask is not None or not relu)):
                vr = valid_rows.to(torch.int32).contiguous() if valid_rows is not None else None
                bnb = BNBwdLink(x3, mask, mean, rstd, vr)
        ctx.save_for_backward(x3, y if mask is None else None, mean, rstd, gamma)
        ctx.relu_mask = mask
        ctx.valid_rows, ctx.relu, ctx.has_res = valid_rows, relu, residual is not None
        ctx.link = link
        ctx.stats = stats
        ctx.ggamma, ctx.gbeta, ctx.shape = ggamma, gbeta, x.shape
        ctx.bnb = bnb
        ctx.planes_on = OPTIONS.planes
        ctx.bwd_in_wgrad = OPTIONS.bn_bwd_in_wgrad
        yo = y.reshape(x.shape)
        if yp is not None:
            _tag_planes(yo, yp.view((K, 2) + tuple(x.shape[1:])), planes >= 2)
        ctx.defer = None
        if be is not ref and planes == 3:
            yo._dls_bn_defer = ctx.defer = defer
        if fold_out is not None:
            yo._dls_res_fold = fold_out
        if bnb is not None:
            yo._dls_bnb = bnb
        return yo

    @staticmethod
    def backward(ctx, dy):
        x3, y, mean, rstd, gamma = ctx.saved_tensors
        be = _be(dy)
        K, R, C = x3.shape
        if ctx.defer is not None:
            ctx.defer.materialize()
            ctx.defer = None
        dy3 = dy.reshape(K, R, C).contiguous()
        if be is ref:
            dx, dgamma, dbeta, dpre = ref.bn_bwd(dy3, x3, y, mean, rstd, gamma, ctx.valid_rows, ctx.relu)
            if ctx.ggamma is not None:
                ctx.ggamma.copy_(dgamma)
                ctx.gbeta.copy_(dbeta)
        else:
            _require_fp32(dy, "batch_norm backward")
            dxm = 2 if (ctx.stats is not None and ctx.stats.dy_planes_ok and ctx.planes_on) else 0
            pre = None
            bnb = ctx.bnb
            if bnb is not None:
                if bnb.part is not None and bnb.key == (dy3.data_ptr(), dy3._version):
                    pre = bnb.part
                bn_bwd_parts_count["used" if pre is not None else "none" if bnb.part is None else "fallback"] += 1
                bnb.part = bnb.key = None
            masked = (ctx.has_res and ctx.link is not None and ctx.relu and ctx.relu_mask is not None
                      and C % 8 == 0)
            if (dxm == 2 and ctx.bwd_in_wgrad and not (ctx.has_res and not masked) and C % 64 == 0
                    and (ctx.relu_mask is not None or not ctx.relu) and x3.is_contiguous()):
                coef = torch.empty((K, C, 3), dtype=torch.float32, device=dy3.device)
                be.bn_bwd(dy3, x3, y, mean, rstd, gamma, ctx.valid_rows, ctx.relu, ctx.ggamma, ctx.gbeta, False,
                          relu_mask=ctx.relu_mask, pre_part=pre, coef_out=coef)
                dx, dxp = be.planes_buffer((K, R, C), dy3.device)
                if masked:
                    ctx.link.grad = MaskedGrad(dy3.view(ctx.shape), ctx.relu_mask)
                dxo = dx.reshape(ctx.shape)
                _tag_planes(dxo, dxp.view((K, 2) + tuple(ctx.shape[1:])), True)
                dxo._dls_bnbwd = DeferredBNBwd(dy3, x3, ctx.relu_mask if ctx.relu else None, coef, ctx.valid_rows,
                                               dxp)
                return dxo, None, None, None, None, None, None, None, None, None, None, None
            out = be.bn_bwd(dy3, x3, y, mean, rstd, gamma, ctx.valid_rows, ctx.relu,
                            ctx.ggamma, ctx.gbeta, ctx.has_res and not masked, relu_mask=ctx.relu_mask,
                            dx_planes=dxm, pre_part=pre)
            dx, dpre = out[0], out[1]
            if masked:
                ctx.link.grad = MaskedGrad(dy3.view(ctx.shape), ctx.relu_mask)
            if dxm:
                dxo = dx.reshape(ctx.shape)
                _tag_planes(dxo, out[2].view((K, 2) + tuple(ctx.shape[1:])), True)
                dres = dpre.reshape(ctx.shape) if (ctx.has_res and not masked) else None
                if dres is not None and ctx.link is not None:
                    ctx.link.grad = dres
                    dres = None
                return dxo, None, None, None, None, None, None, None, dres, None, None, None
            if masked:
                return dx.reshape(ctx.shape), None, None, None, None, None, None, None, None, None, None, None
        dres = dpre.reshape(ctx.shape) if ctx.has_res else None
        if dres is not None and ctx.link is not None:
            ctx.link.grad = dres
            dres = None
        dxo = dx.reshape(ctx.shape)
        if be is not ref:
            dxo._dls_owned = True
        return dxo, None, None, None, None, None, None, None, dres, None, None, None


def batch_norm(x, token, gamma, beta, ggamma, gbeta, valid_rows=None, relu=False, residual=None,
               link: ResidualLink | None = None, stats: BNStats | None = None, planes: int = 0):
    return _BN.apply(x, token, gamma, beta, ggamma, gbeta, valid_rows, relu, residual, link, stats, planes)


class _LN(torch.autograd.Function):
    @staticmethod
    def forward(ctx, x, token, gamma, beta, ggamma, gbeta, planes=False):
        be = _be(x)
        yp = None
        if (planes and OPTIONS.planes and be is not ref and x.dtype == torch.float32
                and be.planes_fit(x[0].numel())):
            y, mean, rstd, yp = be.ln_fwd(x, gamma, beta, planes=True)
        else:
            y, mean, rstd = be.ln_fwd(x, gamma, beta)
        ctx.save_for_backward(x, mean, rstd, gamma)
        ctx.ggamma, ctx.gbeta = ggamma, gbeta
        if yp is not None:
            _tag_planes(y, yp, False)
        return y

    @staticmethod
    def backward(ctx, dy):
        x, mean, rstd, gamma = ctx.saved_tensors
        be = _be(dy)
        dx, dgamma, dbeta = be.ln_bwd(dy.contiguous(), x, mean, rstd, gamma)
        if ctx.ggamma is not None:
            ctx.ggamma.copy_(dgamma)
            ctx.gbeta.copy_(dbeta)
        return dx, None, None, None, None, None, None


def layer_norm(x, token, gamma, beta, ggamma, gbeta, planes: bool = False):
    return _LN.apply(x, token, gamma, beta, ggamma, gbeta, planes)


class _MaxPool(torch.autograd.Function):
    @staticmethod
    def forward(ctx, x, k, s, pad):
        be = _be(x)
        y, idx = be.maxpool_fwd(x, k, s, pad)
        ctx.save_for_backward(idx)
        ctx.k, ctx.s, ctx.pad, ctx.xshape = k, s, pad, x.shape
        return y

    @staticmethod
    def backward(ctx, dy):
        (idx,) = ctx.saved_tensors
        be = _be(dy)
        dx = be.maxpool_bwd(dy.contiguous(), idx, ctx.xshape, ctx.k, ctx.s, ctx.pad)
        return dx, None, None, None


def max_pool2d(x, k, s=None, pad=0):
    return _MaxPool.apply(x, k, s or k, pad)

# ... 313 lines not shown
```

distributed_learning_simulator_amd/ops/hip.py:

```python

from __future__ import annotations

import collections
import importlib
import os
import threading

import torch

from ..options import OPTIONS
from . import ref

try:
    _C = importlib.import_module("distributed_learning_simulator_amd._dls_hip")
except ImportError as e:
    raise ImportError(
        "HIP extension _dls_hip is not built; run `python -m distributed_learning_simulator_amd.ops.build` "
        f"(original error: {e})"
    ) from e


def _check_provenance() -> None:
    from . import build as _build

# ... 251 lines not shown

            acc, acc_mask = MaskedGrad(acc, acc_mask).dense(), None
        if acc_compact:
            full = torch.zeros((K, B, H, W, Ci), dtype=dy.dtype, device=dy.device)
            full[:, :, ::stride, ::stride] = acc
            acc, acc_compact = full, False
        dx = torch.empty((K, B, H, W, Ci), dtype=dy.dtype, device=dy.device)
        for b0, b1 in _batch_chunks(B, per_sample):
            dx[:, b0:b1] = conv_dgrad(dy[:, b0:b1], w, in_hw, stride, pad,
                                      acc=None if acc is None else acc[:, b0:b1].contiguous(), w_split=w_split)
        return dx
    dy, ld_dy = _pix_stride(dy)
    f32 = _f32(dy)
    _check(w, dy.dtype, contiguous=False, name="w")
    assert Co2 == Co
    w_cs, rep = _client_view(w, K)
    dx = torch.empty((K, B, H, W, Ci), dtype=dy.dtype, device=dy.device)
    if acc is not None and not acc_compact:
        assert acc.shape == dx.shape and acc.dtype == dy.dtype and acc.is_contiguous(), acc.shape
    if (not f32 and not acc_compact and ld_dy == Co and (stride == 1 or (gl_mode == 1 and acc is None))
            and _gl(K, B * H * W, Ci, Co, KH * KW)):
        wt = torch.empty((Kw, Ci, KH, KW, Co), dtype=BF16, device=dy.device)
        _C.conv_weight_flip_t(_p(w), _p(wt), w.stride(0), Kw, Co, KH, KW, Ci, _s())
        _C.conv_gl_dgrad(_p(dy), _p(wt), _p(dx), _p(acc), K, rep, B, OH, OW, Co, H, W, Ci, KH, KW, stride, pad, _s())
        return dx
    ws_p, ws_cs, ws_plane = _wsplit_args(w_split if f32 else None, w)
    dyp, dy_cs, dy_lo = _p(dy), dy.stride(0), 0
    if dy_planes is not None and ws_p and planes_ok(Co, Ci, ld_dy):
        dyp, dy_cs, dy_lo = _planes_args(dy_planes, dy)
        planes_launches["dgrad"] += 1
    wt_ready = wt_buf is not None
    if (wt or wt_ready) and _wt_dgrad_ok(Co, Ci, KH, KW, H, W, stride, pad, bool(dy_lo), ws_p):
        if wt_buf is None:
            wt_buf = torch.empty(Kw * 2 * 9 * Ci * Co, dtype=BF16, device=dy.device)
        planes_launches["dgrad_wt"] += 1
    else:
        assert not wt_ready, "conv_dgrad: a prebuilt wt_buf for a dgrad that does not take it"
        wt_buf = None
    _C.conv_dgrad(dyp, _p(w), _p(dx), _p(acc), w_cs, K, rep, B, OH, OW, Co, H, W, Ci, KH, KW, stride, pad,
                  nt_f32_variant if f32 else nt_variant, f32, _s(), ld_dy, dy_cs, ws_p, ws_cs, ws_plane, dy_lo,
                  int(bool(acc_compact)), *bnb_args, _p(wt_buf), _p(acc_mask), int(wt_ready))
    return dx


_part_cache: dict = {}


def _tn_part(numel: int, device) -> torch.Tensor:
    return _grown(_part_cache, (device, torch.cuda.current_stream().cuda_stream), numel, device)


def _sgd_arg(sgd):
    if sgd is None:
        return None
    f, _, off = sgd
    wd, mom, damp, nest = f.hyper
    assert f.theta.stride(1) == 1 and f.mom.stride(0) == f.theta.stride(0) and f.split.is_contiguous()
    return (_p(f.theta) + off * 4, _p(f.mom) + off * 4, _p(f.split) + off * 2, f.theta.stride(0), f.split.stride(0),
            f.split.stride(1), _p(f.lr), _p(f.active), _p(f.first), float(wd), float(mom), float(damp), int(nest))


def _tn_launch(dy, x, gw, dy_cs, x_cs, B, H, W, C, OH, OW, KH, KW, stride, pad, M, Co, R, K, f32, ldy, ldx,
               dy_planes=None, x_planes=None, sgd=None):
    planes = f32 and dy_planes is not None and x_planes is not None
    tv = (_C.conv_tn_pl_variant() if planes else tn_f32_variant) if f32 else tn_variant
    dyp, xp, dy_lo, x_lo = _p(dy), _p(x), 0, 0
    if planes:
        dyp, dy_cs, dy_lo = _planes_args(dy_planes, dy)
        xp, x_cs, x_lo = _planes_args(x_planes, x)
        planes_launches["wgrad"] += 1
    splitk = _C.conv_tn_splitk(K, Co, R, M, C, tv, f32, ldy, ldx, int(planes))
    part = NULL
    if splitk > 1:
        if f32 and (OPTIONS.deterministic or planes):
            part = _p(_tn_part(splitk * K * Co * R, gw.device))
        else:
            gw.zero_()
    if sgd is not None:
        assert planes, "the SGD epilogue needs the plane TN kernels"
    _C.conv_tn(dyp, xp, _p(gw), dy_cs, x_cs, gw.stride(0), B, H, W, C, OH, OW, KH, KW, stride, pad, M, Co, R, K, tv,
               f32, _s(), ldy, ldx, part, dy_lo, x_lo, _sgd_arg(sgd))


def conv_wgrad(dy, x, gw, stride: int, pad: int, dy_planes=None, x_planes=None, sgd=None) -> bool:
    K, B, OH, OW, Co = dy.shape
    _, _, H, W, C = x.shape
    per_sample = max(OH * OW * Co, H * W * C) * dy.element_size()
    if B * per_sample >= WINDOW and dy_planes is None:
        chunks = _batch_chunks(B, per_sample)
        tmp = torch.empty_like(gw) if len(chunks) > 1 else gw
        for i, (b0, b1) in enumerate(chunks):
            conv_wgrad(dy[:, b0:b1], x[:, b0:b1], gw if i == 0 else tmp, stride, pad)
            if i:
                gw.add_(tmp)
        return
    dy, ldy = _pix_stride(dy)
    x, ldx = _pix_stride(x)
    f32 = _f32(dy)
    _check(x, dy.dtype, contiguous=False, name="x")
    assert gw.dtype == torch.float32 and gw.shape[0] == K and gw[0].is_contiguous()
    _, Co2, KH, KW, Ci = gw.shape
    assert Co2 == Co and Ci == C
    M = B * OH * OW
    R = KH * KW * C
    use_pl = (dy_planes is not None and x_planes is not None and f32 and C % 8 == 0 and Co % 8 == 0
              and ldy == Co and ldx == C)
    _tn_launch(dy, x, gw, dy.stride(0), x.stride(0), B, H, W, C, OH, OW, KH, KW, stride, pad, M, Co, R, K, f32,
               ldy, ldx, dy_planes if use_pl else None, x_planes if use_pl else None,
               sgd if use_pl else None)
    return bool(use_pl and sgd is not None)


def halo_wgrad_ok(x_shape, Co: int) -> bool:
    K, B, H, W, C = x_shape
    return bool(_C.halo_wgrad_supported(B, H, W, C, Co))


def halo_wgrad(dy, x, gw, dy_planes=None, x_planes=None, bn=None, valid=None, sgd=None, bn_bwd=None) -> bool:
    K, B, H, W, N = dy.shape
    C = x.shape[-1]
    if x.shape != (K, B, H, W, C) or dy.dtype != F32 or x.dtype != F32 or not halo_wgrad_ok(x.shape, N):
        return False
    assert gw.shape == (K, N, 3, 3, C) and gw.dtype == F32 and gw[0].is_contiguous(), gw.shape
    if gw.data_ptr() % 16 or gw.stride(0) % 4:
        return False
    bnb = None
    if bn_bwd is not None:
        dyo, xb, mk, cf, vr, dxp = bn_bwd
        R = B * H * W
        if not (dyo.is_contiguous() and xb.is_contiguous() and dyo.numel() == K * R * N and xb.numel() == K * R * N
                and dyo.dtype == F32 and xb.dtype == F32):
            return False
        assert cf.shape == (K, N, 3) and cf.dtype == F32 and cf.is_contiguous(), cf.shape
        assert dxp.shape == (K, 2, R, N) and dxp.dtype == BF16 and dxp.is_contiguous(), dxp.shape
        if mk is not None:
            assert mk.dtype == torch.uint8 and mk.is_contiguous() and mk.numel() == K * R * N // 8
        if vr is not None:
            vr = vr.to(torch.int32).contiguous()
            assert vr.shape == (K,)
        bnb = (_p(xb), _p(mk), _p(cf), _p(vr), _p(dxp))
        dyp, dy_cs, dy_lo, dm = _p(dyo), R * N, 0, 2
    elif dy_planes is not None:
        dyp, dy_cs, dy_lo = _planes_args(dy_planes, dy)
        dm = 0
    else:
        if not dy.is_contiguous():
            return False
        dyp, dy_cs, dy_lo, dm = _p(dy), dy.stride(0), 0, 1
    coef, relu, valid_rows_p = NULL, 0, NULL
    if x_planes is not None and bn is None:
        xp, x_cs, x_lo = _planes_args(x_planes, x)
        xm = 0
    else:
        if not x.is_contiguous():
            return False
        xp, x_cs, x_lo, xm = _p(x), x.stride(0), 0, 1
        if bn is not None:
            c, r, v = bn
            assert c.shape == (K, C, 2) and c.dtype == F32 and c.is_contiguous(), c.shape
            coef, relu, xm = _p(c), int(bool(r)), 2
            if v is not None:
                v = v.to(torch.int32).contiguous()
                assert v.shape == (K,)
                valid_rows_p = _p(v)
    n = _C.halo_wgrad_part_floats(K, B, H, W, C, N)
    part = _p(_tn_part(n, dy.device)) if n else NULL
    vimg = NULL
    if valid is not None:
        valid = valid.to(torch.int32).contiguous()
# ... 55 lines not shown
def linear_dgrad(dy, w, gate=None, gate_scale: float = 1.0, w_split=None, dy_planes=None, out_planes: bool = False,
                 acc=None):
    K, N, Fo = dy.shape
    dy = dy.contiguous()
    f32 = _f32(dy)
    Kw, Fo2, Fi = w.shape
    assert w.dtype == dy.dtype
    w_cs, rep = _client_view(w, K)
    dx = torch.empty((K, N, Fi), dtype=dy.dtype, device=dy.device)
    if gate is not None:
        assert gate.shape == dx.shape and gate.dtype == dy.dtype and gate.is_contiguous()
    if acc is not None:
        assert acc.shape == dx.shape and acc.dtype == dy.dtype and acc.is_contiguous()
    ws_p, ws_cs, ws_plane = _wsplit_args(w_split if f32 else None, w)
    dyp, dy_cs, dy_lo = _p(dy), N * Fo, 0
    if dy_planes is not None and f32 and ws_p and planes_ok(Fo, Fi):
        dyp, dy_cs, dy_lo = _planes_args(dy_planes.reshape((K, 2) + tuple(dy.shape[1:])), dy)
        planes_launches["linear_dgrad"] += 1
    xp_, ypp, yp_cs, yp_lo = _out_planes(dx) if (out_planes and f32) else (None, NULL, 0, 0)
    _C.conv_nt(dyp, _p(w), _p(dx), NULL, dy_cs, N * Fi, w_cs, 0, 1, N, 1, Fo, N, 1, 1, 1,
               1, 0, 1, N, Fi, Fo, rep, 0, K, 1, nt_f32_variant if f32 else nt_variant, _p(acc), _p(gate), f32, _s(),
               0, 0, NULL, NULL, NULL, 0.0, float(gate_scale), ws_p, ws_cs, ws_plane, dy_lo, ypp, yp_cs, yp_lo)
    return (dx, xp_) if out_planes else dx


def _drop_seeds(seeds, K: int, p: float):
    if not p:
        return None
    assert seeds is not None and seeds.dtype == torch.int32 and seeds.numel() == K and seeds.is_contiguous()
    return seeds


def dropout_apply(x, seeds, p: float, planes: int = 0, colsum=None):
    K = x.shape[0]
    N = x.shape[-1]
    x = x.contiguous()
    rows = x.numel() // (K * N)
    if planes and _f32(x) and N % 2 == 0:
        if planes == 2:
            out, yp = planes_buffer(tuple(x.shape), x.device)
        else:
            out = torch.empty_like(x)
            yp = torch.empty((K, 2) + tuple(x.shape[1:]), dtype=BF16, device=x.device)
        cs_args = (NULL, 0, NULL)
        if colsum is not None:
            assert colsum.shape == (K, N) and colsum.dtype == F32 and colsum.stride(1) == 1
            ws = _tn_part(_C.dropout_planes_ws_floats(K, rows, N), x.device)
            cs_args = (_p(colsum), colsum.stride(0), _p(ws))
        _C.dropout_planes(_p(x), _p(out) if planes == 1 else NULL, _p(yp), K, rows, N, _p(_drop_seeds(seeds, K, p)),
                          float(p), 1.0 / (1.0 - p), _s(), *cs_args)
        return out, yp
    assert colsum is None, "dropout_apply(colsum=) needs the planes path (fp32, even N)"
    out = torch.empty_like(x)
    _C.dropout_apply(_p(x), _p(out), K, rows, N, N, _p(_drop_seeds(seeds, K, p)), float(p), 1.0 / (1.0 - p),
                     _f32(x), _s())
    return (out, None) if planes else out


def linear_wgrad(dy, x, gw, gb=None, dy_planes=None, x_planes=None, sgd=None) -> bool:
    K, N, Fo = dy.shape
    Fi = x.shape[-1]
    dy = dy.contiguous()
    x = x.contiguous()
    f32 = _f32(dy)
    assert x.dtype == dy.dtype
    assert gw.shape == (K, Fo, Fi) and gw[0].is_contiguous()
    use_pl = dy_planes is not None and x_planes is not None and f32 and Fi % 8 == 0 and Fo % 8 == 0
    dyp = dy_planes.reshape((K, 2) + tuple(dy.shape[1:])) if use_pl else None
    xp = x_planes.reshape((K, 2) + tuple(x.shape[1:])) if use_pl else None
    _tn_launch(dy, x, gw, N * Fo, N * Fi, 1, N, 1, Fi, N, 1, 1, 1, 1, 0, N, Fo, Fi, K, f32, 0, 0, dyp, xp,
               sgd if use_pl else None)
    if gb is not None:
        _col_sum(dy, gb, K, N, Fo)
    return bool(use_pl and sgd is not None)


def planes_buffer(shape, device):
    buf = torch.empty(shape, dtype=F32, device=device)
    K = shape[0]
    return buf, buf.view(K, -1).view(BF16).view((K, 2) + tuple(shape[1:]))


def bn_fwd(x, gamma, beta, valid_rows=None, relu=False, residual=None, eps=1e-5, with_mask=False, pre_stats=None,
           planes: int = 0, res_coef=None):
    K, R, C = x.shape
    x, ldx = _pix_stride(x)
    assert x.stride(0) == R * ldx, "client stride of a strided BN input must be R*ld"
    g_cs, rep = _client_view(gamma, K)
    yp = None
    if planes and x.dtype == F32:
        if planes == 2:
            y, yp = planes_buffer((K, R, C), x.device)
        else:
            y = torch.empty((K, R, C), dtype=x.dtype, device=x.device)
            yp = torch.empty((K, 2, R, C), dtype=BF16, device=x.device)
    else:
        planes = 0
        y = torch.empty((K, R, C), dtype=x.dtype, device=x.device)
    mean = torch.empty((K, C), dtype=torch.float32, device=x.device)
    rstd = torch.empty((K, C), dtype=torch.float32, device=x.device)
    ws = _workspace(_C.bn_workspace_floats(K, R, C), x.device)
    if residual is not None:
        residual = residual.contiguous() if ldx == C else residual
        assert _pix_stride(residual)[1] == ldx and residual.stride() == x.stride()
    vr = valid_rows.to(torch.int32).contiguous() if valid_rows is not None else None
    if pre_stats is not None:
        assert pre_stats.dtype == torch.float32 and pre_stats.is_contiguous()
        assert pre_stats.shape[0] == K and pre_stats.shape[2:] == (2, C), pre_stats.shape
    mask = None
    if with_mask and relu and C % 8 == 0 and ldx % 8 == 0:
        mask = torch.empty((K, R, C // 8), dtype=torch.uint8, device=x.device)
    assert gamma.dtype == x.dtype and (residual is None or residual.dtype == x.dtype)
    if res_coef is not None:
        assert residual is not None and x.dtype == F32 and res_coef.shape == (K, C, 2) and res_coef.is_contiguous()
    _C.bn_fwd(_p(x), _p(gamma), _p(beta), _p(residual), _p(y), _p(mean), _p(rstd), _p(vr), g_cs, K, R, C, int(relu),
              eps, rep, _p(ws), _p(mask), _f32(x), _s(), ldx, _p(pre_stats),
              0 if pre_stats is None else pre_stats.shape[1], _p(yp), int(planes != 2), NULL, 1, _p(res_coef))
    out = (y, mean, rstd, mask) if with_mask else (y, mean, rstd)
    return out + (yp,) if planes else out


def bn_coef(x, gamma, beta, valid_rows=None, eps=1e-5, pre_stats=None):
    K, R, C = x.shape
    assert x.dtype == F32
    x, ldx = _pix_stride(x)
    assert x.stride(0) == R * ldx, "client stride of a strided BN input must be R*ld"
    g_cs, rep = _client_view(gamma, K)
    mean = torch.empty((K, C), dtype=torch.float32, device=x.device)
    rstd = torch.empty((K, C), dtype=torch.float32, device=x.device)
    coef = torch.empty((K, C, 2), dtype=torch.float32, device=x.device)
    ws = _workspace(_C.bn_workspace_floats(K, R, C), x.device)
    vr = valid_rows.to(torch.int32).contiguous() if valid_rows is not None else None
    if pre_stats is not None:
        assert pre_stats.dtype == torch.float32 and pre_stats.is_contiguous()
        assert pre_stats.shape[0] == K and pre_stats.shape[2:] == (2, C), pre_stats.shape
    _C.bn_fwd(_p(x), _p(gamma), _p(beta), NULL, NULL, _p(mean), _p(rstd), _p(vr), g_cs, K, R, C, 0, eps, rep, _p(ws),
              NULL, 1, _s(), ldx, _p(pre_stats),
              0 if pre_stats is None else pre_stats.shape[1], NULL, 1, _p(coef), 0, NULL)
    return coef, mean, rstd


def bn_coef_sums(sums, C: int, gamma, beta, R: int, valid_rows=None, eps=1e-5):
    K = sums.shape[0]
    assert sums.dtype == torch.float64 and sums.is_contiguous() and sums.shape[1] == 2 and C <= sums.shape[2]
    g_cs, rep = _client_view(gamma, K)
    mean = torch.empty((K, C), dtype=torch.float32, device=sums.device)
    rstd = torch.empty((K, C), dtype=torch.float32, device=sums.device)
    coef = torch.empty((K, C, 2), dtype=torch.float32, device=sums.device)
    vr = valid_rows.to(torch.int32).contiguous() if valid_rows is not None else None
    _C.bn_coef_sums(_p(sums), sums.stride(0), sums.shape[2], _p(gamma), _p(beta), _p(vr), g_cs, K, R, C, eps, rep,
                    _p(mean), _p(rstd), _p(coef), _s())
    return coef, mean, rstd


def part_sum_f64(part, out):
    K, nparts, two, g = part.shape
    assert two == 2 and part.dtype == F32 and part.is_contiguous() and 2 * g <= 1024
    assert out.dtype == torch.float64 and out.shape == (K, 2, g) and out.stride(2) == 1
    _C.part_sum_f64(_p(part), K, nparts, g, _p(out), out.stride(0), out.stride(1), _s())


def chan_sums_f64(x, valid_rows, out):
    K, R, C = x.shape
    x, ldx = _pix_stride(x)
    assert x.dtype == F32 and x.stride(0) == R * ldx and 2 * C <= 1024
    assert out.dtype == torch.float64 and out.shape == (K, 2, C) and out.stride(2) == 1
    vr = valid_rows.to(torch.int32).contiguous() if valid_rows is not None else None
    ws = torch.empty(max(1, K * _C.chan_sums_f64_ws(R, C)), dtype=torch.float64, device=x.device)
    _C.chan_sums_f64(_p(x), x.stride(0), ldx, K, R, C, _p(vr), _p(ws), _p(out), out.stride(0), out.stride(1), _s())


def halo_bn_ok(shape, w) -> bool:
    K, B, H, W, C = shape
    return (w.dim() == 5 and w.shape[2] == 3 and w.shape[3] == 3 and w.shape[4] == C
            and bool(_C.conv_halo_bn_supported(B, H, W, C, w.shape[1])))


def bn_apply_only(x, coef, valid_rows, relu: bool, yp, mask=None, y=None):
    K, R, C = x.shape
    assert x.dtype == F32 and x.is_contiguous() and coef.shape == (K, C, 2)
    assert yp is None or (yp.shape == (K, 2, R, C) and yp.dtype == BF16 and yp.is_contiguous())
    assert y is None or (y.shape == (K, R, C) and y.dtype == F32 and y.is_contiguous())
    if mask is not None:
        assert mask.shape == (K, R, C // 8) and C % 8 == 0
    vr = valid_rows.to(torch.int32).contiguous() if valid_rows is not None else None
    _C.bn_apply_only(_p(x), _p(coef), _p(vr), K, R, C, int(relu), _p(yp), _p(mask), _s(), _p(y))


def conv_halo_bn_fwd(x, coef, relu: bool, valid_rows, w, w_split, stats=None, stats_valid=None, yp=None, mask=None):
    K, B, H, W, C = x.shape
    Kw, N, KH, KW, Ci = w.shape
    if not (x.dtype == F32 and x.is_contiguous() and KH == 3 and KW == 3 and Ci == C and w_split is not None):
        return None
    assert coef.shape == (K, C, 2) and coef.dtype == F32 and coef.is_contiguous()
    w_cs, rep = _client_view(w, K)
    ws_p, ws_cs, ws_plane = _wsplit_args(w_split, w)
    y = torch.empty((K, B, H, W, N), dtype=F32, device=x.device)
    vr = valid_rows.to(torch.int32).contiguous() if valid_rows is not None else None
    if stats is not None:
        assert stats.shape == (K, conv_stats_parts(B * H * W), 2, N) and stats.is_contiguous()
# ... 121 lines not shown
    cp = coef
    if C32 != C:
        cp = torch.zeros((K, C32, 2), dtype=F32, device=x.device)
        cp[:, :C].copy_(coef)
    cp = cp.contiguous()
    if w_planes is None:
        w_planes = dense_weight_planes(w)
    assert w_planes.shape == (Kw, 2, N, 3, 3, C32) and w_planes.dtype == BF16 and w_planes.is_contiguous()
    rep = K // Kw
    vr = valid_rows.to(torch.int32).contiguous() if valid_rows is not None else None
    if stats is not None:
        assert stats.shape == (K, conv_stats_parts(B * H * W), 2, N) and stats.is_contiguous()
        if stats_valid is not None:
            stats_valid = stats_valid.to(torch.int32).contiguous()
    if ny is not None:
        assert ny.shape == (K, B * H * W, C) and ny.dtype == F32 and ny.is_contiguous()
    if mask is not None:
        assert ny is not None and C % 8 == 0 and mask.shape == (K, B * H * W, C // 8) and mask.dtype == torch.uint8
        assert mask.is_contiguous()
    ok = _C.conv_halo_bn_dense_fwd(_p(xs), xs.stride(0), ldx, C, _p(cp), int(relu), _p(vr), _p(w_planes),
                                   w_planes.stride(0) if Kw > 1 else 0, w_planes.stride(1), rep, _p(y), y.stride(0),
                                   ldy, K, B, H, W, C32, N, _p(stats), _p(stats_valid), _p(ny),
                                   ny.stride(0) if ny is not None else 0, C, _p(mask), _s())
    if ok:
        planes_launches["fwd_bn_dense"] += 1
    return bool(ok)


def bn_bwd(dy, x, y, mean, rstd, gamma, valid_rows, relu, ggamma, gbeta, need_dpre, relu_mask=None, dx_out=None,
           dx_planes: int = 0, pre_part=None, coef_out=None):
    K, R, C = x.shape
    x, ldx = _pix_stride(x)
    assert x.stride(0) == R * ldx
    dy = dy.contiguous()
    g_cs, rep = _client_view(gamma, K)
    assert rep == 1 or gamma.shape[0] == 1, "bn_bwd supports per-client or fully shared γ"
    if dx_out is not None:
        assert dx_out.shape == (K, R, C) and dx_out.stride() == x.stride() and dx_out.dtype == x.dtype
        dx = dx_out
    else:
        assert ldx == C, "strided x needs a strided dx_out"
    dxp = None
    if dx_planes and dx_out is None and x.dtype == F32:
        if dx_planes == 2:
            dx, dxp = planes_buffer((K, R, C), x.device)
        else:
            dx = torch.empty((K, R, C), dtype=x.dtype, device=x.device)
            dxp = torch.empty((K, 2, R, C), dtype=BF16, device=x.device)
    else:
        dx_planes = 0
        if dx_out is None:
            dx = torch.empty((K, R, C), dtype=x.dtype, device=x.device)
    dpre = torch.empty((K, R, C), dtype=x.dtype, device=x.device) if need_dpre else None
    ws = _workspace(_C.bn_workspace_floats(K, R, C), x.device)
    vr = valid_rows.to(torch.int32).contiguous() if valid_rows is not None else None
    dg_cs = ggamma.stride(0) if ggamma is not None else 0
    assert dy.dtype == x.dtype == gamma.dtype
    if pre_part is not None:
        assert pre_part.dtype == F32 and pre_part.is_contiguous() and pre_part.shape == (K, (R + 31) // 32, 2, C)
    if coef_out is not None:
        assert coef_out.shape == (K, C, 3) and coef_out.dtype == F32 and coef_out.is_contiguous()
        assert dx_out is None and not need_dpre
    _C.bn_bwd(_p(dy), _p(x), _p(y), _p(mean), _p(rstd), _p(gamma), _p(vr), g_cs, K, R, C, int(relu), _p(dx), _p(dpre),
              _p(ggamma), _p(gbeta), dg_cs, _p(ws), _p(relu_mask), _f32(x), _s(), ldx,
              int(dx_out is not None), _p(dxp), int(dx_planes != 2), _p(pre_part),
              0 if pre_part is None else pre_part.shape[1], _p(coef_out), 1 if coef_out is not None else 0)
    if coef_out is not None:
        return None
    if dx_planes:
        return dx, dpre, dxp
    return dx, dpre


def bn_bwd_apply_planes(dy, x, relu_mask, coef, valid_rows, dxp) -> None:
    K, R, C = x.shape
    assert dy.shape == x.shape and dy.is_contiguous() and x.is_contiguous() and dy.dtype == F32 == x.dtype
    assert coef.shape == (K, C, 3) and dxp.shape == (K, 2, R, C) and dxp.is_contiguous()
    ws = _workspace(_C.bn_workspace_floats(K, R, C), x.device)
    vr = valid_rows.to(torch.int32).contiguous() if valid_rows is not None else None
    _C.bn_bwd(_p(dy), _p(x), NULL, NULL, NULL, NULL, _p(vr), 0, K, R, C, int(relu_mask is not None), _p(dxp), NULL,
              NULL, NULL, 0, _p(ws), _p(relu_mask), 1, _s(), C, 0, _p(dxp), 0, NULL, 0, _p(coef), 2)


def ln_fwd(x, gamma, beta, eps=1e-5, planes: bool = False):
    K = x.shape[0]
    C = x.shape[-1]
    x = x.contiguous()
    g_cs, rep = _client_view(gamma, K)
    rpc = x.numel() // (K * C)
    y = torch.empty_like(x)
    mean = torch.empty(x.shape[:-1], dtype=torch.float32, device=x.device)
    rstd = torch.empty_like(mean)
    assert gamma.dtype == x.dtype
    yp = torch.empty((K, 2) + tuple(x.shape[1:]), dtype=BF16, device=x.device) if planes and x.dtype == F32 else None
    _C.ln_fwd(_p(x), _p(gamma), _p(beta), _p(y), _p(mean), _p(rstd), g_cs, K, rpc, C, eps, rep, _f32(x), _s(), _p(yp))
    if planes:
        return y, mean, rstd, yp
    return y, mean, rstd


def ln_bwd(dy, x, mean, rstd, gamma):
    K = x.shape[0]
    C = x.shape[-1]
    assert C <= 1024
    g_cs, rep = _client_view(gamma, K)
    rpc = x.numel() // (K * C)
    dx = torch.empty_like(x)
    if OPTIONS.deterministic:
        dgamma = torch.empty((K, C), dtype=torch.float32, device=x.device)
        dbeta = torch.empty((K, C), dtype=torch.float32, device=x.device)
        ws = _p(_tn_part(_C.ln_workspace_floats(K, rpc, C), x.device))
    else:
        dgamma = torch.zeros((K, C), dtype=torch.float32, device=x.device)
        dbeta = torch.zeros((K, C), dtype=torch.float32, device=x.device)
        ws = NULL
    _C.ln_bwd(_p(dy.contiguous()), _p(x), _p(mean), _p(rstd), _p(gamma), g_cs, K, rpc, C, _p(dx), _p(dgamma),
              _p(dbeta), C, _f32(x), _s(), ws)
    return dx, dgamma, dbeta


def _pool_fwd(x, k, s, pad, mode):
    K, B, H, W, C = x.shape
    x = x.contiguous()
    OH = (H + 2 * pad - k) // s + 1
    OW = (W + 2 * pad - k) // s + 1
    y = torch.empty((K, B, OH, OW, C), dtype=x.dtype, device=x.device)
    idx = torch.empty((K, B, OH, OW, C), dtype=torch.int32, device=x.device) if mode == 0 else None
    _C.pool_fwd(_p(x), _p(y), _p(idx), K, B, H, W, C, OH, OW, k, s, pad, mode, _f32(x), _s())
    return y, idx


def maxpool_fwd(x, k, s, pad=0):
    return _pool_fwd(x, k, s, pad, 0)


def maxpool_bwd(dy, idx, x_shape, k, s, pad=0):
    K, B, H, W, C = x_shape
    _, _, OH, OW, _ = dy.shape
    dx = torch.empty(x_shape, dtype=dy.dtype, device=dy.device)
    _C.pool_bwd(_p(dy.contiguous()), _p(idx), _p(dx), K, B, H, W, C, OH, OW, k, s, pad, 0, _f32(dy), _s())
    return dx


def avgpool_fwd(x, k, s):
    return _pool_fwd(x, k, s, 0, 1)[0]


def avgpool_bwd(dy, x_shape, k, s):
    K, B, H, W, C = x_shape
    _, _, OH, OW, _ = dy.shape
    dx = torch.empty(x_shape, dtype=dy.dtype, device=dy.device)
    _C.pool_bwd(_p(dy.contiguous()), NULL, _p(dx), K, B, H, W, C, OH, OW, k, s, 0, 1, _f32(dy), _s())
    return dx


def gap_fwd(x):
    K, B, H, W, C = x.shape
    x = x.contiguous()
    y = torch.empty((K, B, C), dtype=x.dtype, device=x.device)
    _C.gap_fwd(_p(x), _p(y), K * B, H * W, C, _f32(x), _s())
    return y


def gap_bwd(dy, x_shape):
    K, B, H, W, C = x_shape
    dx = torch.empty(x_shape, dtype=dy.dtype, device=dy.device)
# ... 508 lines not shown
```

distributed_learning_simulator_amd/options.py:

```python

from __future__ import annotations

import contextlib
import dataclasses
import os
import threading


def _env_bool(name: str, default: bool) -> bool:
    v = os.environ.get(name)
    return default if v is None else v not in ("0", "", "false", "False")


def _env_int(name: str, default: int) -> int:
    v = os.environ.get(name)
    return default if v is None or v == "" else int(v)


@dataclasses.dataclass
class RuntimeOptions:
    planes: bool = dataclasses.field(default_factory=lambda: _env_bool("DLS_PLANES", True))
    """BatchNorms emit bf16 (hi, lo) planes for the LDS-DMA plane / halo GEMMs (off: every conv
    splits its operand in registers)."""
    fused_sgd: bool = dataclasses.field(default_factory=lambda: _env_bool("DLS_FUSED_SGD", True))
    """SGD steps of the weights whose plane / halo wgrad kernels can apply them (csrc/sgd_epi.h)
    run in those kernels; the flat step covers the rest (engine.params.FusedSGD)."""
    tfm_planes: bool = dataclasses.field(default_factory=lambda: _env_bool("DLS_TFM_PLANES", True))
    """Transformer split-plane producers: the FFN hidden activation and its gradient (linear1 /
    linear2 epilogues) and the dropout backward of the residual-branch linears (out_proj /
    linear2) write planes for the plane GEMMs (off: fp32 only). (Attention outputs writing planes
    measured +0.4-0.5 s per FedOBD stage-1 round each, profiles/r5_c6_ab_tfm_planes.txt: removed.)"""
    bn_bwd_parts: bool = dataclasses.field(default_factory=lambda: _env_bool("DLS_BN_BWD_PARTS", True))
    """BN backward partial sums from the consuming conv's dgrad epilogue (off: own reduction)."""
    bn_fused_halo: bool = dataclasses.field(default_factory=lambda: _env_bool("DLS_BN_FUSED_HALO", True))
    """A BN(+ReLU) whose only reader is a 3x3 stride-1 conv (ResNet BasicBlock bn1) is applied in
    that conv's halo loader (ops.functional DeferredBN; off: BN apply pass + plane conv)."""
    bn_res_fold: bool = dataclasses.field(default_factory=lambda: _env_bool("DLS_BN_RES_FOLD", True))
    """A ResNet downsample shortcut's BN is applied inside the block's last BN apply, which reads
    its raw input as the residual (ops.functional DeferredRes; off: its own apply pass)."""
    dense_bn_halo: bool = dataclasses.field(default_factory=lambda: _env_bool("DLS_DENSE_BN_HALO", True))
    """DenseNet growth convs apply their BN + ReLU in the halo loader over the block buffer's
    channel prefix (off: BN apply pass + implicit-GEMM conv)."""
    halo_wgrad: bool = dataclasses.field(default_factory=lambda: _env_bool("DLS_HALO_WGRAD", True))
    """3x3 stride-1 weight gradients of 64-512-channel convs (ResNet layers 1-3) on the LDS-halo
    kernel (csrc/conv_halo_wgrad.hip; off: the implicit-GEMM TN kernel)."""
    bn_bwd_in_wgrad: bool = dataclasses.field(default_factory=lambda: _env_bool("DLS_BN_BWD_IN_WGRAD", True))
    """A training BN(+ReLU) whose input gradient feeds only a 3x3 stride-1 conv's backward (ResNet
    BasicBlock bn1 / identity-block bn2, layers 1-3) computes its coefficients only: that conv's halo
    weight gradient applies the BN backward in its dY loader and writes dX's planes for the dgrad
    (ops.functional DeferredBNBwd; off: the BN backward's own apply pass writes them)."""
    dense_wgrad_halo: bool = dataclasses.field(default_factory=lambda: _env_bool("DLS_DENSE_WGRAD_HALO", True))
    """DenseNet growth-conv weight gradients on the LDS-halo kernel (the normalised prefix staged
    once per pixel tile for all nine taps; off: the implicit-GEMM TN kernel)."""
    dense_dgrad_fused: bool = dataclasses.field(default_factory=lambda: _env_bool("DLS_DENSE_DGRAD_FUSED", True))
    """DenseNet growth-conv input gradients fused with the BN backward (csrc/conv_dense_dgrad.hip:
    dX̂ recomputed in a sums pass and an apply pass instead of stored and read twice; off: the
    implicit-GEMM dgrad + the BN backward passes)."""
    dense_y_recompute: bool = dataclasses.field(default_factory=lambda: _env_bool("DLS_DENSE_Y_RECOMPUTE", True))
    """With the fused dgrad and the halo weight gradient, DenseNet training stores no normalised
    activation: both backward kernels rebuild relu(BN(x)) from the raw prefix and the forward's
    (scale, shift), bitwise (off: the forward's halo conv writes it for them)."""
    dense_stats_cache: bool = dataclasses.field(default_factory=lambda: _env_bool("DLS_DENSE_STATS_CACHE", True))
    """DenseNet blocks (fused growth convs) sum each channel's statistics once, from the producing
    conv's epilogue, into running fp64 sums the BN coefficients read (off: a statistics pass over
    the prefix per layer)."""
    deterministic: bool = dataclasses.field(default_factory=lambda: _env_bool("DLS_DETERMINISTIC", True))
    """Split-K weight gradients and column sums folded in a fixed order (off: fp32 atomics)."""
    streams: int = dataclasses.field(default_factory=lambda: _env_int("DLS_STREAMS", 2))
    """Sub-cohort HIP streams trained concurrently on one GPU."""
    ragged_steps: bool = dataclasses.field(default_factory=lambda: _env_bool("DLS_RAGGED_STEPS", True))
    """A cohort's clients are ordered by shard size, so in an epoch's last steps (where only the
    clients with the largest shards still have a batch) the active clients are a row prefix and
    the step runs those rows only (off: every step runs all K rows, idle ones masked)."""
    skip_invalid: bool = dataclasses.field(default_factory=lambda: _env_bool("DLS_SKIP_INVALID", True))
    """Halo convolutions skip the images past a client's valid samples (a partial last batch):
    weight gradients because their dY and X are zeros written by the BatchNorms, forward / dgrad
    tiles whose only readers are BatchNorm passes that stop at the valid rows (off: computed)."""
    graphs: bool = dataclasses.field(default_factory=lambda: _env_bool("DLS_GRAPHS", True))
    """HIP-graph replay of whole training steps (off: eager steps)."""
    max_graphs: int = dataclasses.field(default_factory=lambda: _env_int("DLS_MAX_GRAPHS", 3))
    """Captured step graphs kept per trainer (each owns a private memory pool): a round uses the
    full cohort's and its ragged epoch-end step's (ragged_steps)."""
    eval_max_images: int = dataclasses.field(default_factory=lambda: _env_int("DLS_EVAL_MAX_IMAGES", 4096))
    """Images per evaluation launch (M models x batches): larger launches fill the GPU better and
    cost activation memory; past 4096 they measured slower (GTG utility of 32 models: 38.8 ms per
    model at 4096 vs 39.9 at 8192 and 40.5 at 16384, profiles/r6_c16_eval_max_images.log; the
    headline's one-model test pass equal). Per sub-cohort stream: evaluate() keeps up to `streams` launches in
    flight on separate streams (whose freed blocks the caching allocator does not share), so its
    peak activation memory is about streams x this many images' worth."""
    shared_planes: bool = dataclasses.field(default_factory=lambda: _env_bool("DLS_SHARED_PLANES", True))
    """Shared-model steps (sign-SGD / sync-SGD): every client reads the one shared row's weight
    planes (rep = K) and its activations' planes (off: register-split GEMMs; sign-SGD ResNet-50
    3.51 vs 3.18 s per vote step)."""
    native: dict = dataclasses.field(default_factory=dict)
    """e.g. {"pl_min_wg": 0, "conv_gl": 0, "attn_mfma": 0, "halo_wgrad_unroll": 2}."""


OPTIONS = RuntimeOptions()
_FIELDS = {f.name for f in dataclasses.fields(RuntimeOptions)}


_NATIVE_UNSET = -1000000


def _push_native(native: dict) -> None:
    if not native:
        return
    try:
        from .ops import hip
    except ImportError:
        return
    for k, v in native.items():
        hip._C.set_native_option(str(k), _NATIVE_UNSET if v is None else int(v))


def update(**kw) -> dict:
    old = {}
    for k, v in kw.items():
        if k not in _FIELDS:
            raise KeyError(f"unknown runtime option {k!r}; known: {sorted(_FIELDS)}")
        old[k] = getattr(OPTIONS, k)
        if k == "native":
            merged = dict(OPTIONS.native)
            merged.update(v or {})
            v = {n: x for n, x in merged.items() if x is not None}
        else:
            v = type(old[k])(v)
        setattr(OPTIONS, k, v)
    if "native" in kw:
        _push_native(kw["native"] or {})
    if "skip_invalid" in kw:
        _push_native({"halo_skip": int(OPTIONS.skip_invalid)})
    return old
# ... 54 lines not shown
```

Before: 0.2972 rounds/s.

## Fuse ResNet stem BN apply into its readers and BN backward into wgrad

Defers the CIFAR ResNet stem BN+ReLU so that layer1.0.conv1 applies it in its halo loader and layer1.0.bn2 applies it in its residual fold through a new res_relu path. In backward, the stem BN computes only its coefficients, and the stem conv's fp32 weight-gradient TN kernel applies the BN backward inside its dY loader using the saved input, ReLU mask and coefficients. The goal is to avoid full-size apply passes that write and then re-read large stem activations and gradients. In exchange there are extra loads in the GEMM loader, restricted variants (1 and 5, vector width 8), and an abort if the launch does not match.

Result: faster. 0.3022 rounds/s (median of 6 runs) (+1.7%).

```diff
diff --git a/csrc/bindings.cpp b/csrc/bindings.cpp
--- a/csrc/bindings.cpp
+++ b/csrc/bindings.cpp
@@ -113,6 +113,27 @@
   });
   m.def("conv_nt_num_variants", &conv_nt_num_variants);
   m.def("conv_nt_default_variant", &conv_nt_default_variant);
+  m.def("conv_tn_bn_bwd", [](ptr dy, ptr x, ptr dw, long x_cs, long dw_cs, int B, int H, int W, int C, int OH, int OW,
+                             int KH, int KW, int stride, int pad, int M, int Co, int R, int K, int variant, ptr s,
+                             int ldx, ptr part, ptr bn_x, ptr bn_mask, ptr bn_coef, ptr bn_valid) {
+    ConvTNParams p{};
+    p.part = P<float>(part);
+    p.f32 = 1;
+    p.ldy = Co;
+    p.ldx = ldx;
+    p.dy = P<const bf16_t>(dy);
+    p.x = P<const bf16_t>(x);
+    p.dw = P<float>(dw);
+    p.dy_cs = (long)M * Co; p.x_cs = x_cs; p.dw_cs = dw_cs;
+    p.B = B; p.H = H; p.W = W; p.C = C; p.OH = OH; p.OW = OW; p.KH = KH; p.KW = KW; p.stride = stride; p.pad = pad;
+    p.M = M; p.Co = Co; p.R = R; p.splitk = 1; p.m_per_split = M;
+    p.bnb_x = P<const float>(bn_x);
+    p.bnb_mask = P<const uint8_t>(bn_mask);
+    p.bnb_coef = P<const float>(bn_coef);
+    p.bnb_valid = P<const int>(bn_valid);
+    conv_tn(p, K, variant, S(s));
+  });
+  m.def("conv_tn_f32_bn_bwd_ok", &conv_tn_f32_bn_bwd_ok);
   m.def("conv_tn", [](ptr dy, ptr x, ptr dw, long dy_cs, long x_cs, long dw_cs, int B, int H, int W, int C, int OH,
                       int OW, int KH, int KW, int stride, int pad, int M, int Co, int R, int K, int variant, int f32,
                       ptr s, int ldy, int ldx, ptr part, long dy_lo, long x_lo, py::object sgd) {
@@ -148,12 +169,17 @@
   m.def("bn_workspace_floats", &bn_workspace_floats);
   m.def("bn_fwd", [](ptr x, ptr gamma, ptr beta, ptr res, ptr y, ptr mean, ptr rstd, ptr valid, long g_cs, int K,
                      int R, int C, int relu, float eps, int rep, ptr ws, ptr mask, int f32, ptr s,
-                     int ldx, ptr pre_part, int pre_nparts, ptr yp, int y_f32, ptr coef_out, int apply, ptr res_coef) {
+                     int ldx, ptr pre_part, int pre_nparts, ptr yp, int y_f32, ptr coef_out, int apply, ptr res_coef,
+                     int res_relu) {
     bn_fwd(P<const void>(x), P<const void>(gamma), P<const void>(beta), P<const void>(res), P<void>(y), P<float>(mean),
            P<float>(rstd), P<const int>(valid), g_cs, K, R, C, relu, eps, rep, P<float>(ws), P<uint8_t>(mask),
            f32, S(s), ldx, P<const float>(pre_part), pre_nparts, P<bf16_t>(yp), y_f32,
-           P<float>(coef_out), apply, P<const float>(res_coef));
-  });
+           P<float>(coef_out), apply, P<const float>(res_coef), res_relu);
+  }, py::arg("x"), py::arg("gamma"), py::arg("beta"), py::arg("res"), py::arg("y"), py::arg("mean"), py::arg("rstd"),
+     py::arg("valid"), py::arg("g_cs"), py::arg("K"), py::arg("R"), py::arg("C"), py::arg("relu"), py::arg("eps"),
+     py::arg("rep"), py::arg("ws"), py::arg("mask"), py::arg("f32"), py::arg("s"), py::arg("ldx"),
+     py::arg("pre_part"), py::arg("pre_nparts"), py::arg("yp"), py::arg("y_f32"), py::arg("coef_out"),
+     py::arg("apply"), py::arg("res_coef"), py::arg("res_relu") = 0);
   m.def("conv_halo_bn_supported", &conv_halo_bn_supported);
   m.def("bn_apply_only", [](ptr x, ptr coef, ptr valid, int K, int R, int C, int relu, ptr yp, ptr mask, ptr s, ptr y) {
     bn_apply_only(P<const float>(x), P<const float>(coef), P<const int>(valid), K, R, C, relu, P<bf16_t>(yp),
diff --git a/csrc/conv_f32.hip b/csrc/conv_f32.hip
--- a/csrc/conv_f32.hip
+++ b/csrc/conv_f32.hip
@@ -359,8 +359,9 @@
 int vw(int c) { return (c % 8 == 0) ? 8 : (c % 4 == 0) ? 4 : 1; }
 
 
-template <int BMc, int BNr, int BKT, int WM, int WN, int VA, int VB, int NBUF>
+template <int BMc, int BNr, int BKT, int WM, int WN, int VA, int VB, int NBUF, bool BNB = false>
 __global__ void __launch_bounds__(WM* WN * 64) conv_tn_f32_kernel(ConvTNParams p) {
+  static_assert(!BNB || VA == 8, "the BN-backward loader reads one ReLU mask byte per 8 channels");
   constexpr int T = WM * WN * 64;
   constexpr int TM = BMc / (WM * 32), TN = BNr / (WN * 32);
   constexpr int LDA = BMc + 32;
@@ -409,6 +410,26 @@
   const auto xr = make_rsrc(x, (uint32_t)((long)p.B * p.H * p.W * p.ldx * 4));
   const bool a_live = cok && !(A_PART && tid / CCA >= BKT);
   int k_next = mbeg;
+  constexpr int PAB = BNB ? PA : 1, VAB = BNB ? VA : 1;
+  FV<VAB> rxa[PAB];
+  uint32_t rbits[PAB];
+  bool rlive[PAB];
+  float bn_a[VAB], bn_d[VAB], bn_e[VAB];
+  const auto xbr = make_rsrc(BNB ? p.bnb_x + (long)client * p.dy_cs : reinterpret_cast<const float*>(p.dy),
+                             BNB ? (uint32_t)((long)p.M * p.ldy * 4) : 0u);
+  const uint8_t* __restrict__ bn_mask = nullptr;
+  int a_mend = mend;
+  if constexpr (BNB) {
+#pragma unroll
+    for (int i = 0; i < VA; ++i) {
+      const long q = 3 * ((long)client * p.Co + (cok ? cocol + i : 0));
+      bn_a[i] = p.bnb_coef[q];
+      bn_d[i] = p.bnb_coef[q + 1];
+      bn_e[i] = p.bnb_coef[q + 2];
+    }
+    if (p.bnb_mask) bn_mask = p.bnb_mask + ((long)client * p.M * p.Co >> 3);
+    if (p.bnb_valid) a_mend = min(mend, p.bnb_valid[client]);
+  }
   const int q_b = BKT / (p.OH * p.OW), rem_b = BKT - q_b * p.OH * p.OW;
   const int q_oh = rem_b / p.OW, r_ow = rem_b - q_oh * p.OW;
   const int s_ldx = p.stride * p.ldx, s_row = p.stride * p.W * p.ldx, img = p.H * p.W * p.ldx;
@@ -438,7 +459,16 @@
 #pragma unroll
     for (int j = 0; j < PA; ++j) {
       const int m = k0 + tid / CCA + j * RPA;
-      buf_load<VA>(ra[j].v, dyr, (a_live && m < mend) ? (uint32_t)(a_off + j * a_jstep) * 4u : OOB_OFF);
+      if constexpr (BNB) {
+        const bool live = a_live && m < a_mend;
+        const uint32_t off = live ? (uint32_t)(a_off + j * a_jstep) * 4u : OOB_OFF;
+        buf_load<VA>(ra[j].v, dyr, off);
+        buf_load<VA>(rxa[j].v, xbr, off);
+        rbits[j] = (bn_mask && live) ? bn_mask[(a_off + j * a_jstep) >> 3] : 0xFFu;
+        rlive[j] = live;
+      } else {
+        buf_load<VA>(ra[j].v, dyr, (a_live && m < mend) ? (uint32_t)(a_off + j * a_jstep) * 4u : OOB_OFF);
+      }
     }
     a_off += a_kstep;
 #pragma unroll
@@ -466,6 +496,14 @@
     for (int j = 0; j < PA; ++j) {
       if (A_PART && tid / CCA >= BKT) continue;
       const int off = (buf * BKT + tid / CCA + j * RPA) * LDA + ca * VA;
+      if constexpr (BNB) {
+#pragma unroll
+        for (int i = 0; i < VA; ++i) {
+          const float g = ((rbits[j] >> i) & 1u) ? ra[j].v[i] : 0.f;
+          const float o = fmaf(bn_a[i], g, fmaf(bn_e[i], rxa[j].v[i], bn_d[i]));
+          ra[j].v[i] = rlive[j] ? o : 0.f;
+        }
+      }
       st_split(As + off, As + A_PLANE + off, ra[j]);
     }
 #pragma unroll
@@ -564,6 +602,14 @@
   }
 }
 
+template <int BMc, int BNr, int BKT, int WM, int WN, int NBUF>
+bool launch_tn_f32_bnb(const ConvTNParams& p, int va, int vb, int grid, hipStream_t s) {
+  if (va != 8 || vb != 8) return false;
+  hipLaunchKernelGGL((conv_tn_f32_kernel<BMc, BNr, BKT, WM, WN, 8, 8, NBUF, true>), dim3(grid), dim3(WM * WN * 64), 0,
+                     s, p);
+  return true;
+}
+
 template <int BMc, int BNr, int BKT, int WM, int WN, int NBUF, bool ALLV>
 bool launch_tn_f32_cfg(const ConvTNParams& p, int va, int vb, int grid, hipStream_t s) {
 #define TNF_CASE(A, B)                                                                                          \
@@ -589,7 +635,16 @@
 constexpr int kTnF32Variants = sizeof(kTnF32Tiles) / sizeof(kTnF32Tiles[0]);
 constexpr int TN_BKT_MAX = 32;
 
+bool tn_f32_bnb_variant(int v) { return v == 1 || v == 5; }
+
 bool launch_tn_f32_variant(int v, const ConvTNParams& p, int va, int vb, int grid, hipStream_t s) {
+  if (p.bnb_coef) {
+    switch (v) {
+      case 1: return launch_tn_f32_bnb<64, 128, 32, 2, 2, 2>(p, va, vb, grid, s);
+      case 5: return launch_tn_f32_bnb<64, 64, 32, 2, 2, 2>(p, va, vb, grid, s);
+      default: return false;
+    }
+  }
   switch (v) {
     case 0: return launch_tn_f32_cfg<128, 128, 32, 2, 2, 2, true>(p, va, vb, grid, s);
     case 1: return launch_tn_f32_cfg<64, 128, 32, 2, 2, 2, true>(p, va, vb, grid, s);
@@ -708,6 +763,12 @@
   const int va = vw(std::gcd(p.Co, p.ldy));
   const int vb = vw(std::gcd(p.C, p.ldx));
   variant = resolve_tn_f32_variant(variant, K, p.Co, p.R, va, vb);
+  if (p.bnb_coef && !(p.bnb_x && p.ldy == p.Co && p.dy_cs == (long)p.M * p.Co && va == 8 && vb == 8 &&
+                      tn_f32_bnb_variant(variant))) {
+    fprintf(stderr, "conv_tn_f32: the BN-backward loader does not serve this launch (Co %d, C %d, variant %d)\n",
+            p.Co, p.C, variant);
+    abort();
+  }
   tn_f32_split(K, p.Co, p.R, p.M, variant, p.splitk, p.m_per_split);
   const TnTile t = kTnF32Tiles[variant];
   const long tiles = (long)K * cdiv(p.Co, t.bm) * cdiv(p.R, t.bn);
@@ -716,6 +777,11 @@
   if (p.splitk > 1 && p.part != nullptr) tn_fold(p.part, p.dw, p.dw_cs, K, p.splitk, (long)p.Co * p.R, s);
 }
 
+bool conv_tn_f32_bn_bwd_ok(int K, int Co, int R, int gco, int gc, int variant) {
+  const int va = vw(gco), vb = vw(gc);
+  return va == 8 && vb == 8 && tn_f32_bnb_variant(resolve_tn_f32_variant(variant, K, Co, R, va, vb));
+}
+
 int conv_tn_f32_splitk(int K, int Co, int R, int M, int gco, int gc, int variant) {
   int splitk, mps;
   variant = resolve_tn_f32_variant(variant, K, Co, R, vw(gco), vw(gc));
diff --git a/csrc/dls.h b/csrc/dls.h
--- a/csrc/dls.h
+++ b/csrc/dls.h
@@ -190,6 +190,10 @@
   long dy_lo, x_lo;
   SgdEpi sgd;
   int pix;
+  const float* bnb_x;
+  const uint8_t* bnb_mask;
+  const float* bnb_coef;
+  const int* bnb_valid;
 };
 
 struct ConvGLParams {
@@ -287,6 +291,7 @@
              const SgdEpi* sgd = nullptr);
 int conv_tn_f32_num_variants();
 int conv_tn_f32_splitk(int K, int Co, int R, int M, int gco, int gc, int variant);
+bool conv_tn_f32_bn_bwd_ok(int K, int Co, int R, int gco, int gc, int variant);
 
 long bn_workspace_floats(int K, long R, int C);
 void bn_fwd(const void* x, const void* gamma, const void* beta, const void* res, void* y, float* mean, float* rstd,
@@ -295,7 +300,8 @@
             int ldx = 0, const float* pre_part = nullptr,
             int pre_nparts = 0, bf16_t* yp = nullptr,
             int y_f32 = 1, float* coef_out = nullptr, int apply = 1,
-            const float* res_coef = nullptr);
+            const float* res_coef = nullptr,
+            int res_relu = 0);
 void bn_bwd(const void* dy, const void* x, const void* y, const float* mean, const float* rstd, const void* gamma,
             const int* valid_rows, long g_cs, int K, int R, int C, int relu, void* dx, void* dpre, float* dgamma,
             float* dbeta, long dg_cs, float* ws, const uint8_t* relu_mask, int f32,
diff --git a/csrc/norm.hip b/csrc/norm.hip
--- a/csrc/norm.hip
+++ b/csrc/norm.hip
@@ -350,7 +350,7 @@
                                                        const float* __restrict__ coef, int R, int C, int relu,
                                                        int rpb, uint8_t* __restrict__ rmask, int ldx,
                                                        bf16_t* __restrict__ yp, int y_f32,
-                                                       const float* __restrict__ res_coef) {
+                                                       const float* __restrict__ res_coef, int res_relu) {
   const int k = blockIdx.y;
   const int CT = C / V;
   const int nvalid = valid_rows ? min(valid_rows[k], R) : R;
@@ -382,7 +382,10 @@
         if (res) {
           float rv[V];
           load_vec<V>(res + offx, rv);
-          if (res_coef) {
+          if (res_coef && res_relu) {
+#pragma unroll
+            for (int j = 0; j < V; ++j) out[j] += fmaxf(fmaf(rv[j], rsc[j], rsh[j]), 0.f);
+          } else if (res_coef) {
 #pragma unroll
             for (int j = 0; j < V; ++j) out[j] += fmaf(rv[j], rsc[j], rsh[j]);
           } else {
@@ -706,7 +709,8 @@
 void bn_fwd(const void* x, const void* gamma, const void* beta, const void* res, void* y, float* mean, float* rstd,
             const int* valid_rows, long g_cs, int K, int R, int C, int relu, float eps, int rep, float* ws,
             uint8_t* rmask, int f32, hipStream_t s, int ldx, const float* pre_part,
-            int pre_nparts, bf16_t* yp, int y_f32, float* coef_out, int apply, const float* res_coef) {
+            int pre_nparts, bf16_t* yp, int y_f32, float* coef_out, int apply, const float* res_coef,
+            int res_relu) {
   if (ldx == 0) ldx = C;
   float* coef = coef_out ? coef_out : ws;
   const float* part = pre_part ? pre_part : ws + (long)3 * C * K;
@@ -737,7 +741,7 @@
     if (apply) {
       DISPATCH_V(V, hipLaunchKernelGGL((bn_apply_kernel<TT, VV>), grid, dim3(256), 0, s, CP(x), CP(res), MP(y),
                                        valid_rows, coef, R, C, relu, rpb, rmask, ldx, f32 ? yp : nullptr,
-                                       f32 ? y_f32 : 1, res_coef));
+                                       f32 ? y_f32 : 1, res_coef, res_relu));
     }
   });
 }
@@ -748,10 +752,11 @@
   dim3 grid(cdiv(R, rpb), K);
   if (C % 8 == 0) {
     hipLaunchKernelGGL((bn_apply_kernel<float, 8>), grid, dim3(256), 0, s, x, (const float*)nullptr, y,
-                       valid_rows, coef, R, C, relu, rpb, rmask, C, yp, y ? 1 : 0, (const float*)nullptr);
+                       valid_rows, coef, R, C, relu, rpb, rmask, C, yp, y ? 1 : 0, (const float*)nullptr, 0);
   } else {
     hipLaunchKernelGGL((bn_apply_kernel<float, 1>), grid, dim3(256), 0, s, x, (const float*)nullptr, y,
-                       valid_rows, coef, R, C, relu, rpb, (uint8_t*)nullptr, C, yp, y ? 1 : 0, (const float*)nullptr);
+                       valid_rows, coef, R, C, relu, rpb, (uint8_t*)nullptr, C, yp, y ? 1 : 0, (const float*)nullptr,
+                       0);
   }
 }
 
diff --git a/distributed_learning_simulator_amd/models/zoo.py b/distributed_learning_simulator_amd/models/zoo.py
--- a/distributed_learning_simulator_amd/models/zoo.py
+++ b/distributed_learning_simulator_amd/models/zoo.py
@@ -161,10 +161,12 @@
         self.child("fc", Linear(c, classes))
 
     def forward(self, x, ctx):
-        x = conv_bn(self.conv1, self.bn1, x, ctx, planes=0 if not self.cifar_stem else 1)
+        blocks = [b for s in self.stages for b in s.children]
+        first = blocks[0] if blocks else None
+        two_reader = self.cifar_stem and isinstance(first, BasicBlock) and first.down is None
+        x = conv_bn(self.conv1, self.bn1, x, ctx, planes=0 if not self.cifar_stem else 5 if two_reader else 1)
         if not self.cifar_stem:
             x = self.maxpool.forward(x, ctx)
-        blocks = [b for s in self.stages for b in s.children]
         for i, b in enumerate(blocks):
             nxt = blocks[i + 1] if i + 1 < len(blocks) else None
             op = 0 if nxt is None else 2 if nxt.down is not None else 1
diff --git a/distributed_learning_simulator_amd/ops/functional.py b/distributed_learning_simulator_amd/ops/functional.py
--- a/distributed_learning_simulator_amd/ops/functional.py
+++ b/distributed_learning_simulator_amd/ops/functional.py
@@ -43,12 +43,13 @@
 
 class BNStats:
 
-    __slots__ = ("valid", "part", "dy_planes_ok")
+    __slots__ = ("valid", "part", "dy_planes_ok", "wgrad_bn_bwd_ok")
 
     def __init__(self, valid=None):
         self.valid = valid
         self.part = None
         self.dy_planes_ok = False
+        self.wgrad_bn_bwd_ok = False
 
 
 bn_bwd_parts_count = {"used": 0, "none": 0, "fallback": 0}
@@ -101,6 +102,32 @@
             self.pending = False
 
 
+stem_defer_count = {"conv": 0, "res": 0, "materialized": 0}
+
+
+class DeferredStemBN(DeferredBN):
+
+    __slots__ = ("y32",)
+
+    def __init__(self, x, coef, relu, valid_rows, yp, mask, write_out):
+        super().__init__(x, coef, relu, valid_rows, yp, mask, write_out)
+        self.y32 = None
+
+    def materialize(self):
+        if self.pending:
+            stem_defer_count["materialized"] += 1
+        super().materialize()
+
+    def materialize_f32(self):
+        if self.y32 is None:
+            from . import hip
+
+            self.y32 = torch.empty(self.x.shape, dtype=self.x.dtype, device=self.x.device)
+            hip.bn_apply_only(self.x, self.coef, self.valid_rows, self.relu, None, y=self.y32)
+            stem_defer_count["materialized"] += 1
+        return self.y32
+
+
 res_fold_count = {"folded": 0, "materialized": 0}
 
 
@@ -142,6 +169,32 @@
 
     def wgrad_args(self):
         return (self.dy, self.x, self.mask, self.coef, self.valid_rows, self.dxp)
+
+
+bn_bwd_f32_defer_count = {"wgrad": 0, "materialized": 0}
+
+
+class DeferredBNBwdF32:
+
+    __slots__ = ("dy", "x", "mask", "coef", "valid_rows", "dx", "pending")
+
+    def __init__(self, dy, x, mask, coef, valid_rows, dx):
+        self.dy, self.x, self.mask, self.coef, self.valid_rows, self.dx = dy, x, mask, coef, valid_rows, dx
+        self.pending = True
+
+    def materialize(self, holder=None):
+        if self.pending:
+            from . import hip
+
+            hip.bn_bwd_apply_f32(self.dy, self.x, self.mask, self.coef, self.valid_rows, self.dx)
+            self.pending = False
+            bn_bwd_f32_defer_count["materialized"] += 1
+        for t in (self.dx, holder):
+            if t is not None:
+                t._dls_planes_only = False
+
+    def wgrad_args(self):
+        return (self.dy, self.x, self.mask, self.coef, self.valid_rows)
 
 
 class _Conv(torch.autograd.Function):
@@ -179,8 +232,8 @@
         ctx.bn_src = None
         defer = getattr(x, "_dls_bn_defer", None)
         if defer is not None and defer.pending:
-            if (use_pl and stride == 1 and pad == 1 and KH == 3 and w.shape[3] == 3 and b is None
-                    and be.halo_bn_ok(x.shape, w)):
+            if (OPTIONS.bn_fused_halo and use_pl and stride == 1 and pad == 1 and KH == 3 and w.shape[3] == 3
+                    and b is None and be.halo_bn_ok(x.shape, w)):
                 part = (torch.empty((K, be.conv_stats_parts(B * OH * OW), 2, w.shape[1]), dtype=torch.float32,
                                     device=x.device) if want_stats else None)
                 bn_wgrad = (defer.write_out and gw is not None and OPTIONS.halo_wgrad
@@ -191,6 +244,8 @@
                                         mask=defer.mask if defer.write_out else None)
                 if y is not None:
                     defer.pending = False
+                    if isinstance(defer, DeferredStemBN):
+                        stem_defer_count["conv"] += 1
                     if want_stats:
                         stats.part = part
                     if bn_wgrad:
@@ -207,6 +262,13 @@
             y = be.conv_fwd(x, w, stride, pad, bias=b, w_split=w_split, **pl)
         else:
             y = be.conv_fwd(x, w, stride, pad, bias=b)
+        ctx.wgrad_bn_bwd = bool(
+            OPTIONS.bn_bwd_in_wgrad_f32 and stats is not None and be is not ref and x.dtype == torch.float32
+            and not ctx.needs_input_grad[0] and link is None and donor is None and b is None and gw is not None
+            and not use_pl and not big and w.shape[1] % 8 == 0 and x.is_contiguous()
+            and be.conv_wgrad_bn_bwd_ok(x.shape, w.shape[1], KH, w.shape[3]))
+        if stats is not None:
+            stats.wgrad_bn_bwd_ok = ctx.wgrad_bn_bwd
         ctx.w_split = w_split
         ctx.expect_dy_planes = stats is not None and stats.dy_planes_ok
         ctx.x_planes_only = bool(getattr(x, "_dls_planes_only", False))
@@ -227,7 +289,7 @@
         return y
 
     @staticmethod
-    def _wgrad(ctx, dy, x, w, dyp, be, bbd=None, sgd_ok=True) -> bool:
+    def _wgrad(ctx, dy, x, w, dyp, be, bbd=None, sgd_ok=True, bbf=None) -> bool:
         if bbd is not None:
             if not (ctx.stride == 1 and ctx.pad == 1 and w.shape[2] == 3 and w.shape[3] == 3):
                 return False
@@ -246,7 +308,9 @@
         sgd = ctx.sgd if not padded else None
         stepped = False
         gw = torch.empty((K,) + tuple(w.shape[1:]), dtype=torch.float32, device=dy.device) if padded else ctx.gw
-        if be is ref:
+        if bbf is not None:
+            be.conv_wgrad(dy, x, gw, ctx.stride, ctx.pad, bn_bwd=bbf.wgrad_args())
+        elif be is ref:
             gw.copy_(ref.conv_wgrad(dy.float(), x.float(), (K,) + tuple(w.shape[1:]), ctx.stride, ctx.pad))
             if ctx.gb is not None:
                 ctx.gb.copy_(dy.float().sum(dim=(1, 2, 3)))
@@ -319,12 +383,22 @@
                 bn_bwd_defer_count["wgrad"] += 1
             else:
                 bbd.materialize()
+        bbf = getattr(dy, "_dls_bnbwd_f32", None)
+        if bbf is not None and bbf.pending:
+            if ctx.wgrad_bn_bwd and not ctx.needs_input_grad[0] and acc is None and dyp is None:
+                _Conv._wgrad(ctx, dy, x, w, None, be, bbf=bbf)
+                wgrad_done = True
+                bbf.pending = False
+                bn_bwd_f32_defer_count["wgrad"] += 1
+            else:
+                bbf.materialize(dy)
         if dyp is not None and ctx.xp is None:
             raise RuntimeError("conv2d backward: dY planes without the input's planes")
         if dyp is None:
             if ctx.expect_dy_planes:
                 raise RuntimeError("conv2d backward: the BN wrote dY as planes only, but they did not arrive")
-            _require_fp32(dy, "conv2d backward")
+            if not wgrad_done or ctx.needs_input_grad[0]:
+                _require_fp32(dy, "conv2d backward")
         donor = ctx.donor
         compact = (donor is not None and not donor.receiver_done and be is not ref and dy.dtype == torch.float32
                    and ctx.stride > 1 and ctx.pad == 0 and w.shape[2] == 1 and w.shape[3] == 1 and acc is None
@@ -545,14 +619,24 @@
         K = x.shape[0]
         C = x.shape[-1]
         _require_fp32(x, "batch_norm")
-        if residual is not None:
+        x3 = x.reshape(K, -1, C)
+        res_coef = None
+        res_relu = False
+        r3 = None
+        sdef = getattr(residual, "_dls_bn_defer", None) if residual is not None else None
+        if isinstance(sdef, DeferredStemBN):
+            if (be is not ref and x.dtype == torch.float32 and sdef.y32 is None and sdef.valid_rows is valid_rows
+                    and sdef.x.shape == x3.shape and x3.is_contiguous() and sdef.x.is_contiguous()):
+                r3, res_coef, res_relu = sdef.x, sdef.coef, sdef.relu
+                stem_defer_count["res"] += 1
+            else:
+                r3 = sdef.materialize_f32().reshape(K, -1, C)
+        elif residual is not None:
             _require_fp32(residual, "batch_norm residual")
-        x3 = x.reshape(K, -1, C)
-        r3 = residual.reshape(K, -1, C) if residual is not None else None
+            r3 = residual.reshape(K, -1, C)
         mask = None
         yp = None
         bnb = None
-        res_coef = None
         fold = getattr(residual, "_dls_res_fold", None) if residual is not None else None
         if fold is not None and fold.pending:
             if (be is not ref and x.dtype == torch.float32 and fold.valid_rows is valid_rows
@@ -575,21 +659,24 @@
                 planes = 2
             if planes == 4 and not (OPTIONS.bn_res_fold and residual is None and not relu and x3.is_contiguous()):
                 planes = 0
+            if planes == 5 and not (OPTIONS.bn_stem_defer and residual is None and C8 and x3.is_contiguous()):
+                planes = 1
             if planes == 4:
                 coef, mean, rstd = be.bn_coef(x3, gamma, beta, valid_rows, pre_stats=pre)
                 y = torch.empty((K, x3.shape[1], C), dtype=x.dtype, device=x.device)
                 fold_out = DeferredRes(x3, coef, valid_rows, y)
                 defer = None
                 planes = 0
-            elif planes == 3:
+            elif planes == 3 or planes == 5:
                 coef, mean, rstd = be.bn_coef(x3, gamma, beta, valid_rows, pre_stats=pre)
                 y, yp = be.planes_buffer((K, x3.shape[1], C), x.device)
                 mask = torch.empty((K, x3.shape[1], C // 8), dtype=torch.uint8, device=x.device) if (wm and relu) else None
-                defer = DeferredBN(x3, coef, relu, valid_rows, yp, mask, write_out=wm)
+                defer = (DeferredBN if planes == 3 else DeferredStemBN)(x3, coef, relu, valid_rows, yp, mask,
+                                                                        write_out=wm)
             else:
                 defer = None
                 out = be.bn_fwd(x3, gamma, beta, valid_rows, relu, r3, with_mask=wm, pre_stats=pre, planes=planes,
-                                res_coef=res_coef)
+                                res_coef=res_coef, res_relu=res_relu)
                 y, mean, rstd = out[:3]
                 mask = out[3] if wm else None
                 if planes:
@@ -609,11 +696,12 @@
         ctx.bnb = bnb
         ctx.planes_on = OPTIONS.planes
         ctx.bwd_in_wgrad = OPTIONS.bn_bwd_in_wgrad
+        ctx.bwd_in_wgrad_f32 = OPTIONS.bn_bwd_in_wgrad_f32
         yo = y.reshape(x.shape)
         if yp is not None:
             _tag_planes(yo, yp.view((K, 2) + tuple(x.shape[1:])), planes >= 2)
         ctx.defer = None
-        if be is not ref and planes == 3:
+        if be is not ref and planes in (3, 5):
             yo._dls_bn_defer = ctx.defer = defer
         if fold_out is not None:
             yo._dls_res_fold = fold_out
@@ -659,6 +747,19 @@
                 _tag_planes(dxo, dxp.view((K, 2) + tuple(ctx.shape[1:])), True)
                 dxo._dls_bnbwd = DeferredBNBwd(dy3, x3, ctx.relu_mask if ctx.relu else None, coef, ctx.valid_rows,
                                                dxp)
+                return dxo, None, None, None, None, None, None, None, None, None, None, None
+            if (dxm == 0 and ctx.bwd_in_wgrad_f32 and ctx.stats is not None and ctx.stats.wgrad_bn_bwd_ok
+                    and not ctx.has_res and C % 8 == 0 and (ctx.relu_mask is not None or not ctx.relu)
+                    and x3.is_contiguous() and dy3.dtype == torch.float32):
+                coef = torch.empty((K, C, 3), dtype=torch.float32, device=dy3.device)
+                be.bn_bwd(dy3, x3, y, mean, rstd, gamma, ctx.valid_rows, ctx.relu, ctx.ggamma, ctx.gbeta, False,
+                          relu_mask=ctx.relu_mask, pre_part=pre, coef_out=coef)
+                dx = torch.empty((K, R, C), dtype=torch.float32, device=dy3.device)
+                dxo = dx.reshape(ctx.shape)
+                _tag_planes(dxo, None, True)
+                _tag_planes(dx, None, True)
+                dxo._dls_bnbwd_f32 = DeferredBNBwdF32(dy3, x3, ctx.relu_mask if ctx.relu else None, coef,
+                                                      ctx.valid_rows, dx)
                 return dxo, None, None, None, None, None, None, None, None, None, None, None
             out = be.bn_bwd(dy3, x3, y, mean, rstd, gamma, ctx.valid_rows, ctx.relu,
                             ctx.ggamma, ctx.gbeta, ctx.has_res and not masked, relu_mask=ctx.relu_mask,
diff --git a/distributed_learning_simulator_amd/ops/hip.py b/distributed_learning_simulator_amd/ops/hip.py
--- a/distributed_learning_simulator_amd/ops/hip.py
+++ b/distributed_learning_simulator_amd/ops/hip.py
@@ -357,9 +357,44 @@
                f32, _s(), ldy, ldx, part, dy_lo, x_lo, _sgd_arg(sgd))
 
 
-def conv_wgrad(dy, x, gw, stride: int, pad: int, dy_planes=None, x_planes=None, sgd=None) -> bool:
+def conv_wgrad_bn_bwd_ok(x_shape, Co: int, KH: int, KW: int, x_dtype=F32) -> bool:
+    K, B, H, W, C = x_shape
+    if x_dtype != F32 or Co % 8 or C % 8:
+        return False
+    return bool(_C.conv_tn_f32_bn_bwd_ok(K, Co, KH * KW * C, Co, C, tn_f32_variant))
+
+
+def conv_wgrad(dy, x, gw, stride: int, pad: int, dy_planes=None, x_planes=None, sgd=None, bn_bwd=None) -> bool:
     K, B, OH, OW, Co = dy.shape
     _, _, H, W, C = x.shape
+    if bn_bwd is not None:
+        dyo, xb, mk, cf, vr = bn_bwd
+        M = B * OH * OW
+        assert dy_planes is None and x_planes is None and sgd is None and dy.dtype == F32 and x.dtype == F32
+        assert max(M * Co, B * H * W * C) * 4 < WINDOW and x.is_contiguous()
+        assert conv_wgrad_bn_bwd_ok(x.shape, Co, gw.shape[2], gw.shape[3])
+        assert dyo.dtype == F32 and xb.dtype == F32 and dyo.is_contiguous() and xb.is_contiguous()
+        assert dyo.numel() == K * M * Co and xb.numel() == K * M * Co
+        assert cf.shape == (K, Co, 3) and cf.dtype == F32 and cf.is_contiguous(), cf.shape
+        if mk is not None:
+            assert mk.dtype == torch.uint8 and mk.is_contiguous() and mk.numel() == K * M * Co // 8
+        if vr is not None:
+            vr = vr.to(torch.int32).contiguous()
+            assert vr.shape == (K,)
+        assert gw.dtype == torch.float32 and gw.shape[0] == K and gw[0].is_contiguous()
+        _, Co2, KH, KW, Ci = gw.shape
+        assert Co2 == Co and Ci == C
+        R = KH * KW * C
+        splitk = _C.conv_tn_splitk(K, Co, R, M, C, tn_f32_variant, 1, Co, C, 0)
+        part = NULL
+        if splitk > 1:
+            if OPTIONS.deterministic:
+                part = _p(_tn_part(splitk * K * Co * R, gw.device))
+            else:
+                gw.zero_()
+        _C.conv_tn_bn_bwd(_p(dyo), _p(x), _p(gw), x.stride(0), gw.stride(0), B, H, W, C, OH, OW, KH, KW, stride, pad, M,
+                          Co, R, K, tn_f32_variant, _s(), C, part, _p(xb), _p(mk), _p(cf), _p(vr))
+        return False
     per_sample = max(OH * OW * Co, H * W * C) * dy.element_size()
     if B * per_sample >= WINDOW and dy_planes is None:
         chunks = _batch_chunks(B, per_sample)
@@ -581,7 +616,7 @@
 
 
 def bn_fwd(x, gamma, beta, valid_rows=None, relu=False, residual=None, eps=1e-5, with_mask=False, pre_stats=None,
-           planes: int = 0, res_coef=None):
+           planes: int = 0, res_coef=None, res_relu: bool = False):
     K, R, C = x.shape
     x, ldx = _pix_stride(x)
     assert x.stride(0) == R * ldx, "client stride of a strided BN input must be R*ld"
@@ -612,9 +647,11 @@
     assert gamma.dtype == x.dtype and (residual is None or residual.dtype == x.dtype)
     if res_coef is not None:
         assert residual is not None and x.dtype == F32 and res_coef.shape == (K, C, 2) and res_coef.is_contiguous()
+    assert res_coef is not None or not res_relu, "res_relu needs res_coef"
     _C.bn_fwd(_p(x), _p(gamma), _p(beta), _p(residual), _p(y), _p(mean), _p(rstd), _p(vr), g_cs, K, R, C, int(relu),
               eps, rep, _p(ws), _p(mask), _f32(x), _s(), ldx, _p(pre_stats),
-              0 if pre_stats is None else pre_stats.shape[1], _p(yp), int(planes != 2), NULL, 1, _p(res_coef))
+              0 if pre_stats is None else pre_stats.shape[1], _p(yp), int(planes != 2), NULL, 1, _p(res_coef),
+              int(bool(res_relu)))
     out = (y, mean, rstd, mask) if with_mask else (y, mean, rstd)
     return out + (yp,) if planes else out
 
@@ -902,6 +939,16 @@
               NULL, NULL, 0, _p(ws), _p(relu_mask), 1, _s(), C, 0, _p(dxp), 0, NULL, 0, _p(coef), 2)
 
 
+def bn_bwd_apply_f32(dy, x, relu_mask, coef, valid_rows, dx) -> None:
+    K, R, C = x.shape
+    assert dy.shape == x.shape and dy.is_contiguous() and x.is_contiguous() and dy.dtype == F32 == x.dtype
+    assert coef.shape == (K, C, 3) and dx.shape == (K, R, C) and dx.dtype == F32 and dx.is_contiguous()
+    ws = _workspace(_C.bn_workspace_floats(K, R, C), x.device)
+    vr = valid_rows.to(torch.int32).contiguous() if valid_rows is not None else None
+    _C.bn_bwd(_p(dy), _p(x), NULL, NULL, NULL, NULL, _p(vr), 0, K, R, C, int(relu_mask is not None), _p(dx), NULL,
+              NULL, NULL, 0, _p(ws), _p(relu_mask), 1, _s(), C, 0, NULL, 1, NULL, 0, _p(coef), 2)
+
+
 def ln_fwd(x, gamma, beta, eps=1e-5, planes: bool = False):
     K = x.shape[0]
     C = x.shape[-1]
diff --git a/distributed_learning_simulator_amd/options.py b/distributed_learning_simulator_amd/options.py
--- a/distributed_learning_simulator_amd/options.py
+++ b/distributed_learning_simulator_amd/options.py
@@ -38,6 +38,10 @@
     bn_res_fold: bool = dataclasses.field(default_factory=lambda: _env_bool("DLS_BN_RES_FOLD", True))
     """A ResNet downsample shortcut's BN is applied inside the block's last BN apply, which reads
     its raw input as the residual (ops.functional DeferredRes; off: its own apply pass)."""
+    bn_stem_defer: bool = dataclasses.field(default_factory=lambda: _env_bool("DLS_BN_STEM_DEFER", True))
+    """The CIFAR ResNet stem BN(+ReLU), read by layer1.0.conv1 (planes) and by layer1.0.bn2 (fp32, as
+    its identity residual), is applied by those two readers: the conv in its halo loader, the BN
+    in its residual fold (ops.functional DeferredStemBN; off: one apply pass writes both forms)."""
     dense_bn_halo: bool = dataclasses.field(default_factory=lambda: _env_bool("DLS_DENSE_BN_HALO", True))
     """DenseNet growth convs apply their BN + ReLU in the halo loader over the block buffer's
     channel prefix (off: BN apply pass + implicit-GEMM conv)."""
@@ -49,6 +53,11 @@
     BasicBlock bn1 / identity-block bn2, layers 1-3) computes its coefficients only: that conv's halo
     weight gradient applies the BN backward in its dY loader and writes dX's planes for the dgrad
     (ops.functional DeferredBNBwd; off: the BN backward's own apply pass writes them)."""
+    bn_bwd_in_wgrad_f32: bool = dataclasses.field(default_factory=lambda: _env_bool("DLS_BN_BWD_IN_WGRAD_F32", True))
+    """A training BN(+ReLU) behind a conv whose input needs no gradient (the ResNet stem) computes
+    its backward coefficients only: the conv's fp32 weight gradient applies the BN backward in its dY
+    loader (ops.functional DeferredBNBwdF32, csrc/conv_f32.hip; off: the BN backward's own apply pass
+    writes dX and the weight gradient reads it back)."""
     dense_wgrad_halo: bool = dataclasses.field(default_factory=lambda: _env_bool("DLS_DENSE_WGRAD_HALO", True))
     """DenseNet growth-conv weight gradients on the LDS-halo kernel (the normalised prefix staged
     once per pixel tile for all nine taps; off: the implicit-GEMM TN kernel)."""
```
